# Enigmatisms/NeRF

Hardware: AMD Instinct MI355X
Metric: rays/s (64+128 samples), 800x800 (higher is better)
Workload: dtype bf16

## Files before the change

### include/nerf_amd.h

```cpp
#ifndef NERF_AMD_H
#define NERF_AMD_H

#include <stddef.h>
#include <stdint.h>

#ifdef __cplusplus
extern "C" {
#endif

#define NERF_AMD_OK            0
#define NERF_AMD_EINVAL       -1
#define NERF_AMD_EUNSUPPORTED -2
#define NERF_AMD_EHIP         -3

#define NERF_AMD_F32   0
#define NERF_AMD_BF16  1
#define NERF_AMD_BF16_F8 2

#define NERF_AMD_NET_PROPOSAL 0
#define NERF_AMD_NET_MIP      1
#define NERF_AMD_NET_REF      2
#define NERF_AMD_NET_PROPOSAL_128 3
#define NERF_AMD_PROP_W128 0x100
#define NERF_AMD_NET_MIP_128 4
// ... 100 lines not shown
                      int softplus_density, float blur_alpha, uint64_t rng_seed, int64_t rng_ray_offset,
                      float* z_fine, int64_t* below, float* w_prop, float* z_coarse, void* stream);

int nerf_amd_composite(const float* rgbo, const float* z, int z_stride, const float* dirs, int dirs_stride,
                       int64_t N, int S, int flags, int act, float sigma_shift, float near, float far,
                       const float* normal, const float* cam_dir,
                       float* rgb, float* weights, float* depth, float* normal_img, void* stream);

int nerf_amd_merge_depths(const float* z_fine, const float* z_coarse, int64_t N, int K, int C, float* z_out, void* stream);

int nerf_amd_merge_depths_order(const float* z_fine, const float* z_coarse, const int64_t* f_inds, int64_t N, int K, int C, float* z_out,
                                int64_t* order, int64_t* all_inds, void* stream);

int nerf_amd_coarse_grad_select(const float* grads, const int64_t* sort_inds, int64_t N, int T, int D, int c_pnum, float* out, void* stream);

#define NERF_AMD_DOT_LOSS_WORKSPACE_FLOATS 512
int nerf_amd_weighted_dot_loss(const float* w, const float* a, const float* b, int64_t M, int mode, float scale, float* out, float* workspace, void* stream);
int nerf_amd_weighted_dot_loss_backward(const float* g, const float* w, const float* a, const float* b, int64_t M, int mode, float scale, float* d_w,
                                        float* d_a, float* d_b, void* stream);

#define NERF_AMD_DISTORTION_MAX_S 1024
#define NERF_AMD_DISTORTION_WORKSPACE_FLOATS 4096
int nerf_amd_distortion_loss(const float* w, const float* t, int64_t N, int S, int mode, float scale, float* out, float* workspace, void* stream);
int nerf_amd_distortion_loss_backward(const float* w, const float* t, int64_t N, int S, int mode, float scale, const float* g, float* d_w,
                                      float* d_t, void* stream);

int nerf_amd_mfma_stream(int iters, int workgroups, int mode, float* sink, void* stream);

int nerf_amd_get_bounds(const float* w_prop, const int64_t* below, int64_t N, int C, int K, float* bounds, void* stream);

size_t nerf_amd_train_dump_bytes(int net, int precision, int64_t M);
int nerf_amd_proposal_forward_train(const void* packed, int precision, const nerf_amd_samples* src, float* density, void* dump,
                                    void* stream);
int nerf_amd_mip_forward_train(const void* packed, int precision, const nerf_amd_samples* src, float* rgbo, void* dump, void* stream);
int nerf_amd_train_dump_to_rows(const void* dump, int net, int precision, int64_t M, int layer, int n_features, void* out,
                                void* stream);
int nerf_amd_relu_mask(void* delta, const void* act, int precision, int64_t n, void* stream);
int64_t nerf_amd_relu_mask_bias_partials(int precision, int64_t rows, int cols);
int nerf_amd_relu_mask_bias(void* delta, const void* act, int precision, int64_t rows, int cols, float* col_sum, void* stream);

int64_t nerf_amd_train_dump_rows_mask_partials(void);
int nerf_amd_train_dump_rows_mask(const void* dump, int net, int precision, int64_t M, int layer, int n_features, void* act_out, void* delta,
                                  float* col_sum, void* stream);

int nerf_amd_encode_rows(const float* x, int x_stride, int64_t M, int L, int normalize, int precision, void* out, void* stream);

size_t nerf_amd_packed_backward_bytes(int net, int precision);
int    nerf_amd_pack_weights_backward(int net, int precision, const float* const* weights, int n_tensors, void* packed_bwd, void* stream);
int    nerf_amd_proposal_backward_chain(const void* packed_bwd, int precision, const float* g_density, int64_t M, const void* act_dump,
                                        void* delta_dump, void* stream);
int    nerf_amd_mip_backward_chain(const void* packed_bwd, int precision, const float* g_rgbo, const float* rgbo, int64_t M,
                                   const void* act_dump, void* delta_dump, void* stream);
size_t nerf_amd_weight_grads_workspace_bytes(int net, int precision, int64_t M);
int    nerf_amd_proposal_weight_grads(int precision, int64_t M, const void* act_dump, const void* delta_dump, float* const* d_weights,
                                      float* const* d_biases, void* workspace, void* stream);
int    nerf_amd_mip_weight_grads(int precision, int64_t M, const void* act_dump, const void* delta_dump, const float* const* weights,
                                 const float* const* biases, float* const* d_weights, float* const* d_biases, void* workspace, void* stream);
int    nerf_amd_ref_forward_train_dump(const void* packed, int precision, const nerf_amd_samples* src, int ref_flags, const float* bn_noise,
                                       float* rgbo, float* normal, void* dump, float* aux, void* stream);
int    nerf_amd_ref_forward_train_dump_rng(const void* packed, int precision, const nerf_amd_samples* src, int ref_flags, uint64_t noise_seed,
                                           const uint64_t* noise_seed_dev, float noise_std, float* rgbo, float* normal, void* dump, float* aux,
                                           void* stream);
int    nerf_amd_philox_normal(float* out, int64_t M, uint64_t rng_seed, const uint64_t* seed_dev, float std, int64_t sample_offset, void* stream);
#define NERF_AMD_CONTRACTED 0x100
size_t nerf_amd_density_grad_workspace_bytes(int net, int precision, int64_t M);
int    nerf_amd_density_grad(int net, const void* packed_bwd, int precision, int64_t M, const void* act_dump, const float* x, int x_stride,
                             const float* scale, int scale_stride, float* grad, void* workspace, void* stream);
size_t nerf_amd_ref_backward_workspace_bytes(int precision, int64_t M);
int    nerf_amd_ref_backward(const void* packed_bwd, int precision, int ref_flags, int64_t M, const void* act_dump, const float* aux,
                             const float* dirs, int dir_stride, const float* g_out, int g_stride, const float* ide_table,
                             float* const* d_weights, float* const* d_biases, void* workspace, void* stream);
int    nerf_amd_adam_step(float* const* params, const float* const* grads, float* const* exp_avg, float* const* exp_avg_sq,
                          const int64_t* numel, int n_tensors, float* step, double lr, const double* lr_dev, double beta1, double beta2,
                          double eps, float grad_scale, void* stream);

int nerf_amd_sigma_to_weights_backward(const float* sigma, const float* z, const float* dirs, int64_t N, int S, int act,
                                       const float* d_weights, float* d_sigma, void* stream);
int nerf_amd_composite_backward(const float* rgbo, const float* z, int z_stride, const float* dirs, int dirs_stride, int64_t N, int S,
                                int flags, int act, float sigma_shift, float near, float far, const float* d_rgb,
                                const float* d_weights, const float* d_depth, float* d_rgbo, void* stream);
int nerf_amd_max_blur_backward(const float* weights, const float* d_out, int64_t N, int S, float* d_weights, void* stream);
int nerf_amd_get_bounds_backward(const int64_t* below, const float* d_bounds, int64_t N, int C, int K, float* d_w_prop, void* stream);

size_t nerf_amd_render_workspace_bytes(int64_t N, int n_fine);
int    nerf_amd_render_rays(const void* packed_prop, const void* packed_mip, int precision,
                            const float* rays, const nerf_amd_samples* camera, int64_t ray_offset,
                            const float* z_base, const float* u_strat, const float* u_inv, int64_t N, int n_fine,
                            float near, float far, int white_bkg,
                            float* rgb, float* depth, float* weights, void* workspace, void* stream);

size_t nerf_amd_render_ref_workspace_bytes(int64_t N, int n_fine);
int    nerf_amd_render_rays_ref(const void* packed_prop, const void* packed_ref, int precision, int ref_flags, const float* rays,
                                const nerf_amd_samples* camera, int64_t ray_offset, const float* z_base, const float* u_strat,
                                const float* u_inv, int64_t N, int n_fine, float near, float far, int white_bkg, const float* cam_dir,
                                float* rgb, float* depth, float* normal_img, void* workspace, void* stream);

size_t nerf_amd_gemm_workspace_bytes(int64_t M, int64_t N, int64_t P);
int    nerf_amd_gemm(int precision, int64_t M, int64_t N, int64_t P, const float* A, int64_t a_si, int64_t a_sp,
                     const float* B, int64_t b_sp, int64_t b_sj, float* C, int64_t ldc, const float* bias, int act,
                     const float* mask, int64_t ldm, void* workspace, void* stream);
int    nerf_amd_sigmoid_backward(const float* g, int64_t g_stride, const float* y, int64_t y_stride, int64_t M, int cols,
                                 float* out, int64_t out_stride, void* stream);

int nerf_amd_ref_dir_inputs(const float* heads, int64_t heads_stride, const float* dirs, int64_t dirs_stride, int64_t M, int ide_level,
                            const float* ide_table, float* out, int64_t out_stride, float* normal, void* stream);
int nerf_amd_ref_dir_inputs_backward(const float* heads, int64_t heads_stride, const float* dirs, int64_t dirs_stride, int64_t M, int ide_level,
                                     const float* ide_table, const float* d_out, int64_t d_out_stride, const float* g_normal,
                                     int64_t g_normal_stride, float* d_heads, int64_t d_heads_stride, void* stream);
int nerf_amd_ref_combine(const float* heads, int64_t heads_stride, const float* spec, int64_t spec_stride, int64_t M, int ref_flags,
                         float* rgbo, void* stream);
int nerf_amd_ref_combine_backward(const float* g_rgbo, int64_t g_stride, const float* heads, int64_t heads_stride, const float* spec,
                                  int64_t spec_stride, int64_t M, int ref_flags, float* d_spec, int64_t d_spec_stride, float* d_heads,
                                  int64_t d_heads_stride, void* stream);
int nerf_amd_positional_encoding_backward(const float* d_enc, int64_t d_enc_stride, const float* x, int64_t x_stride, int64_t M, int L,
                                          int cat_origin, float* d_x, void* stream);
int nerf_amd_add_rows(float* dst, int64_t dst_stride, const float* src, int64_t src_stride, int64_t M, int cols, void* stream);
int nerf_amd_contract_positions(const float* x, int64_t x_stride, int64_t M, const float* g, int64_t g_stride, float* out, void* stream);

int nerf_amd_rows_gemm(int64_t M, int64_t N, int64_t K, const void* X, int64_t ldx, const void* W, int64_t ldw, int64_t n_pad,
                       const float* bias, int act, void* C, int64_t ldc, int out_bf16, void* stream);
int nerf_amd_rows_to_bf16(const float* src, int64_t rows_src, int64_t src_stride, int64_t rows, int cols, int fill, void* dst,
                          int64_t dst_stride, void* stream);

#ifdef __cplusplus
}
#endif
#endif
```

### nerf_amd/_lib.py

```python
import ctypes as C
import os

import torch

_HERE = os.path.dirname(os.path.abspath(__file__))
LIB_PATH = os.environ.get("NERF_AMD_LIB") or os.path.join(_HERE, "libnerf_amd.so")

F32, BF16 = 0, 1
BF16_F8 = 2
EXPECTED_VERSION = 125
NET_PROPOSAL, NET_MIP, NET_REF, NET_PROPOSAL_128, NET_MIP_128 = 0, 1, 2, 3, 4
FINE_W128 = 0x200
PROP_W128 = 0x100
ACT_RELU, ACT_IDENTITY, ACT_SOFTPLUS = 0, 1, 2

c_float_p = C.POINTER(C.c_float)
c_void = C.c_void_p
i64 = C.c_int64


class Samples(C.Structure):
    _fields_ = [("mode", C.c_int32), ("S", C.c_int32), ("M", C.c_int64), ("pts", c_void), ("pts_stride", C.c_int32),
                ("z_stride", C.c_int32), ("rays", c_void), ("z", c_void), ("z_base", c_void), ("u", c_void),
                ("z_jitter", C.c_float), ("H", C.c_int32), ("W", C.c_int32), ("fx", C.c_float), ("fy", C.c_float),
# ... 5 lines not shown
    "nerf_amd_last_error": (C.c_char_p, []),
    "nerf_amd_version": (C.c_int, []),
    "nerf_amd_device_info": (C.c_int, [C.POINTER(C.c_int), C.POINTER(C.c_int)]),
    "nerf_amd_packed_bytes": (C.c_size_t, [C.c_int, C.c_int]),
    "nerf_amd_pack_weights": (C.c_int, [C.c_int, C.c_int, C.POINTER(c_void), C.POINTER(c_void), C.c_int, c_void, c_void]),
    "nerf_amd_proposal_forward": (C.c_int, [c_void, C.c_int, C.POINTER(Samples), c_void, c_void]),
    "nerf_amd_mip_forward": (C.c_int, [c_void, C.c_int, C.POINTER(Samples), c_void, c_void]),
    "nerf_amd_mip_forward_composite": (C.c_int, [c_void, C.c_int, C.POINTER(Samples), C.c_int, C.c_float, C.c_float, c_void, c_void, c_void,
                                                 c_void]),
    "nerf_amd_ref_forward": (C.c_int, [c_void, C.c_int, C.POINTER(Samples), C.c_int, c_void, c_void, c_void]),
    "nerf_amd_ref_forward_train": (C.c_int, [c_void, C.c_int, C.POINTER(Samples), C.c_int, c_void, c_void, c_void, c_void]),
    "nerf_amd_positional_encoding": (C.c_int, [c_void, i64, C.c_int, c_void, c_void]),
    "nerf_amd_ipe_feature": (C.c_int, [c_void, c_void, i64, C.c_int, C.c_int, C.c_float, c_void, c_void, c_void, c_void, c_void]),
    "nerf_amd_ipe_feature_contracted": (C.c_int, [c_void, c_void, i64, C.c_int, C.c_int, C.c_float, c_void, c_void, c_void, c_void, c_void]),
    "nerf_amd_cone_parameters": (C.c_int, [c_void, i64, C.c_int, C.c_float, c_void, c_void, c_void, c_void]),
    "nerf_amd_dirs_norm": (C.c_int, [c_void, i64, c_void, c_void]),
    "nerf_amd_generate_rays": (C.c_int, [c_float_p, C.c_int, C.c_int, C.c_float, C.c_float, i64, i64, c_void, c_void]),
    "nerf_amd_length2pts": (C.c_int, [c_void, c_void, i64, C.c_int, c_void, c_void]),
    "nerf_amd_sigma_to_weights": (C.c_int, [c_void, c_void, c_void, i64, C.c_int, C.c_int, c_void, c_void]),
    "nerf_amd_max_blur": (C.c_int, [c_void, i64, C.c_int, C.c_float, c_void, c_void]),
    "nerf_amd_inverse_sample": (C.c_int, [c_void, c_void, c_void, i64, C.c_int, C.c_int, C.c_int, c_void, c_void, c_void]),
    "nerf_amd_sample_pdf": (C.c_int, [c_void, c_void, c_void, i64, C.c_int, C.c_int, c_void, c_void, c_void, c_void]),
    "nerf_amd_pixel_rays": (C.c_int, [c_float_p, C.c_float, C.c_float, c_void, i64, c_void, c_void]),
    "nerf_amd_sample_training_rays": (C.c_int, [c_void, c_void, i64, c_float_p, C.c_float, C.c_float, C.c_float, C.c_float, i64, C.c_int, C.c_uint64,
                                               c_void, c_void, c_void, c_void, c_void]),
    "nerf_amd_sample_training_rays_dev": (C.c_int, [c_void, c_void, i64, c_void, C.c_float, C.c_float, C.c_float, C.c_float, i64, C.c_int, c_void,
                                                   c_void, c_void, c_void, c_void, c_void]),
    "nerf_amd_sample_scene_rays": (C.c_int, [c_void, c_void, i64, C.c_int, C.c_int, c_void, i64, C.c_int, C.c_int, C.c_int, C.c_int, C.c_float, C.c_float,
                                            C.c_float, C.c_float, i64, C.c_int, C.c_uint64, c_void, c_void, c_void, c_void, c_void, c_void, c_void]),
    "nerf_amd_philox_uniforms": (C.c_int, [c_void, i64, C.c_int, C.c_uint64, c_void, c_void]),
    "nerf_amd_philox_stream": (C.c_int, [c_void, i64, C.c_int, C.c_uint64, c_void, i64, C.c_int, c_void]),
    "nerf_amd_advance_seed": (C.c_int, [c_void, c_void]),
    "nerf_amd_stratified_points": (C.c_int, [c_void, c_void, c_void, C.c_float, i64, C.c_int, c_void, c_void, c_void]),
    "nerf_amd_resample": (C.c_int, [c_void, c_void, c_void, c_void, C.c_float, c_void, C.c_int, c_void, i64, C.c_int,
                                    C.c_int, C.c_int, C.c_float, C.c_uint64, i64, c_void, c_void, c_void, c_void, c_void]),
    "nerf_amd_composite": (C.c_int, [c_void, c_void, C.c_int, c_void, C.c_int, i64, C.c_int, C.c_int, C.c_int, C.c_float, C.c_float,
                                     C.c_float, c_void, c_void, c_void, c_void, c_void, c_void, c_void]),
    "nerf_amd_train_dump_rows_mask_partials": (i64, []),
    "nerf_amd_train_dump_rows_mask": (C.c_int, [c_void, C.c_int, C.c_int, i64, C.c_int, C.c_int, c_void, c_void, c_void, c_void]),
    "nerf_amd_render_ref_workspace_bytes": (C.c_size_t, [i64, C.c_int]),
    "nerf_amd_render_rays_ref": (C.c_int, [c_void, c_void, C.c_int, C.c_int, c_void, C.POINTER(Samples), i64, c_void, c_void, c_void, i64, C.c_int,
                                          C.c_float, C.c_float, C.c_int, c_void, c_void, c_void, c_void, c_void, c_void]),
    "nerf_amd_encode_rows": (C.c_int, [c_void, C.c_int, i64, C.c_int, C.c_int, C.c_int, c_void, c_void]),
    "nerf_amd_merge_depths": (C.c_int, [c_void, c_void, i64, C.c_int, C.c_int, c_void, c_void]),
    "nerf_amd_merge_depths_order": (C.c_int, [c_void, c_void, c_void, i64, C.c_int, C.c_int, c_void, c_void, c_void, c_void]),
    "nerf_amd_coarse_grad_select": (C.c_int, [c_void, c_void, i64, C.c_int, C.c_int, C.c_int, c_void, c_void]),
    "nerf_amd_mfma_stream": (C.c_int, [C.c_int, C.c_int, C.c_int, c_void, c_void]),
    "nerf_amd_weighted_dot_loss": (C.c_int, [c_void, c_void, c_void, i64, C.c_int, C.c_float, c_void, c_void, c_void]),
    "nerf_amd_weighted_dot_loss_backward": (C.c_int, [c_void, c_void, c_void, c_void, i64, C.c_int, C.c_float, c_void, c_void, c_void, c_void]),
    "nerf_amd_distortion_loss": (C.c_int, [c_void, c_void, i64, C.c_int, C.c_int, C.c_float, c_void, c_void, c_void]),
    "nerf_amd_distortion_loss_backward": (C.c_int, [c_void, c_void, i64, C.c_int, C.c_int, C.c_float, c_void, c_void, c_void, c_void]),
    "nerf_amd_get_bounds": (C.c_int, [c_void, c_void, i64, C.c_int, C.c_int, c_void, c_void]),
    "nerf_amd_train_dump_bytes": (C.c_size_t, [C.c_int, C.c_int, i64]),
    "nerf_amd_proposal_forward_train": (C.c_int, [c_void, C.c_int, C.POINTER(Samples), c_void, c_void, c_void]),
    "nerf_amd_mip_forward_train": (C.c_int, [c_void, C.c_int, C.POINTER(Samples), c_void, c_void, c_void]),
    "nerf_amd_train_dump_to_rows": (C.c_int, [c_void, C.c_int, C.c_int, i64, C.c_int, C.c_int, c_void, c_void]),
    "nerf_amd_relu_mask": (C.c_int, [c_void, c_void, C.c_int, i64, c_void]),
    "nerf_amd_relu_mask_bias_partials": (i64, [C.c_int, i64, C.c_int]),
    "nerf_amd_relu_mask_bias": (C.c_int, [c_void, c_void, C.c_int, i64, C.c_int, c_void, c_void]),
    "nerf_amd_packed_backward_bytes": (C.c_size_t, [C.c_int, C.c_int]),
    "nerf_amd_pack_weights_backward": (C.c_int, [C.c_int, C.c_int, C.POINTER(c_void), C.c_int, c_void, c_void]),
    "nerf_amd_proposal_backward_chain": (C.c_int, [c_void, C.c_int, c_void, i64, c_void, c_void, c_void]),
    "nerf_amd_mip_backward_chain": (C.c_int, [c_void, C.c_int, c_void, c_void, i64, c_void, c_void, c_void]),
    "nerf_amd_weight_grads_workspace_bytes": (C.c_size_t, [C.c_int, C.c_int, i64]),
    "nerf_amd_proposal_weight_grads": (C.c_int, [C.c_int, i64, c_void, c_void, C.POINTER(c_void), C.POINTER(c_void), c_void, c_void]),
    "nerf_amd_mip_weight_grads": (C.c_int, [C.c_int, i64, c_void, c_void, C.POINTER(c_void), C.POINTER(c_void), C.POINTER(c_void),
                                           C.POINTER(c_void), c_void, c_void]),
    "nerf_amd_ref_forward_train_dump": (C.c_int, [c_void, C.c_int, C.POINTER(Samples), C.c_int, c_void, c_void, c_void, c_void, c_void, c_void]),
    "nerf_amd_ref_forward_train_dump_rng": (C.c_int, [c_void, C.c_int, C.POINTER(Samples), C.c_int, C.c_uint64, c_void, C.c_float, c_void, c_void, c_void,
                                                      c_void, c_void]),
    "nerf_amd_philox_normal": (C.c_int, [c_void, i64, C.c_uint64, c_void, C.c_float, i64, c_void]),
    "nerf_amd_density_grad_workspace_bytes": (C.c_size_t, [C.c_int, C.c_int, i64]),
    "nerf_amd_density_grad": (C.c_int, [C.c_int, c_void, C.c_int, i64, c_void, c_void, C.c_int, c_void, C.c_int, c_void, c_void, c_void]),
    "nerf_amd_ref_backward_workspace_bytes": (C.c_size_t, [C.c_int, i64]),
    "nerf_amd_ref_backward": (C.c_int, [c_void, C.c_int, C.c_int, i64, c_void, c_void, c_void, C.c_int, c_void, C.c_int, c_void, C.POINTER(c_void),
                                       C.POINTER(c_void), c_void, c_void]),
    "nerf_amd_adam_step": (C.c_int, [C.POINTER(c_void), C.POINTER(c_void), C.POINTER(c_void), C.POINTER(c_void), C.POINTER(i64), C.c_int, c_void,
                                    C.c_double, c_void, C.c_double, C.c_double, C.c_double, C.c_float, c_void]),
    "nerf_amd_sigma_to_weights_backward": (C.c_int, [c_void, c_void, c_void, i64, C.c_int, C.c_int, c_void, c_void, c_void]),
    "nerf_amd_composite_backward": (C.c_int, [c_void, c_void, C.c_int, c_void, C.c_int, i64, C.c_int, C.c_int, C.c_int, C.c_float, C.c_float,
                                              C.c_float, c_void, c_void, c_void, c_void, c_void]),
    "nerf_amd_max_blur_backward": (C.c_int, [c_void, c_void, i64, C.c_int, c_void, c_void]),
    "nerf_amd_get_bounds_backward": (C.c_int, [c_void, c_void, i64, C.c_int, C.c_int, c_void, c_void]),
    "nerf_amd_render_workspace_bytes": (C.c_size_t, [i64, C.c_int]),
    "nerf_amd_render_rays": (C.c_int, [c_void, c_void, C.c_int, c_void, C.POINTER(Samples), i64, c_void, c_void, c_void, i64,
                                       C.c_int, C.c_float, C.c_float, C.c_int, c_void, c_void, c_void, c_void, c_void]),
    "nerf_amd_gemm_workspace_bytes": (C.c_size_t, [i64, i64, i64]),
    "nerf_amd_gemm": (C.c_int, [C.c_int, i64, i64, i64, c_void, i64, i64, c_void, i64, i64, c_void, i64, c_void, C.c_int, c_void, i64, c_void, c_void]),
    "nerf_amd_sigmoid_backward": (C.c_int, [c_void, i64, c_void, i64, i64, C.c_int, c_void, i64, c_void]),
    "nerf_amd_ref_dir_inputs": (C.c_int, [c_void, i64, c_void, i64, i64, C.c_int, c_void, c_void, i64, c_void, c_void]),
    "nerf_amd_ref_dir_inputs_backward": (C.c_int, [c_void, i64, c_void, i64, i64, C.c_int, c_void, c_void, i64, c_void, i64, c_void, i64, c_void]),
    "nerf_amd_ref_combine": (C.c_int, [c_void, i64, c_void, i64, i64, C.c_int, c_void, c_void]),
    "nerf_amd_ref_combine_backward": (C.c_int, [c_void, i64, c_void, i64, c_void, i64, i64, C.c_int, c_void, i64, c_void, i64, c_void]),
    "nerf_amd_positional_encoding_backward": (C.c_int, [c_void, i64, c_void, i64, i64, C.c_int, C.c_int, c_void, c_void]),
    "nerf_amd_contract_positions": (C.c_int, [c_void, i64, i64, c_void, i64, c_void, c_void]),
    "nerf_amd_add_rows": (C.c_int, [c_void, i64, c_void, i64, i64, C.c_int, c_void]),
    "nerf_amd_rows_gemm": (C.c_int, [i64, i64, i64, c_void, i64, c_void, i64, i64, c_void, C.c_int, c_void, i64, C.c_int, c_void]),
    "nerf_amd_rows_to_bf16": (C.c_int, [c_void, i64, i64, i64, C.c_int, C.c_int, c_void, i64, c_void]),
}


def _load():
    if not os.path.exists(LIB_PATH):
        raise ImportError(
            "nerf_amd: %s is missing. Build it with `python -c 'import __graft_entry__ as g; g.build()'` "
            "(or `make -C nerf_amd/csrc`). There is no CPU/torch fallback." % LIB_PATH)
    lib = C.CDLL(LIB_PATH)
    for name, (res, args) in SIGNATURES.items():
        fn = getattr(lib, name)
        fn.restype = res
        fn.argtypes = args
    got = lib.nerf_amd_version()
    if got != EXPECTED_VERSION and not os.environ.get("NERF_AMD_LIB"):
        raise ImportError("nerf_amd: %s is ABI version %d, this package expects %d -- rebuild it (`make -C nerf_amd/csrc`)" % (LIB_PATH, got, EXPECTED_VERSION))
    return lib


lib = _load()


class NerfAmdError(RuntimeError):
    pass


def check(rc: int, what: str = ""):
    if rc != 0:
        msg = lib.nerf_amd_last_error()
        raise NerfAmdError("%s failed (%d): %s" % (what or "nerf_amd call", rc, msg.decode() if msg else "?"))
```

### nerf_amd/csrc/capi.hip

```cpp
#include <hip/hip_runtime.h>
#include <stdio.h>
#include <string.h>

#include "../../include/nerf_amd.h"
#include "mlp_layout.h"

int mlp_launch_proposal(const void*, int, const nerf_amd_samples&, float*, hipStream_t);
int mlp_launch_proposal128(const void*, int, const nerf_amd_samples&, float*, hipStream_t);
int mlp_launch_mip(const void*, int, const nerf_amd_samples&, float*, hipStream_t);
int mlp_launch_mip128(const void*, int, const nerf_amd_samples&, float*, hipStream_t);
int mlp_launch_mip_composite(const void*, int, const nerf_amd_samples&, float*, float*, float*, int, float, float, hipStream_t);
int mlp_launch_ref(const void*, int, const nerf_amd_samples&, float*, float*, const float*, int, hipStream_t);
size_t mlp_train_layer_stride(int, int64_t);
size_t mlp_train_mask_stride(int, int64_t);
int mlp_launch_proposal_train(const void*, int, const nerf_amd_samples&, float*, void*, hipStream_t);
int mlp_launch_mip_train(const void*, int, const nerf_amd_samples&, float*, void*, hipStream_t);
int sk_frag_to_rows(const void*, int, int64_t, int, int64_t, void*, hipStream_t);
int sk_relu_mask(void*, const void*, int, int64_t, hipStream_t);
int sk_merge_sorted(const float*, const float*, int64_t, int, int, float*, hipStream_t);
int sk_merge_sorted_order(const float*, const float*, const int64_t*, int64_t, int, int, float*, int64_t*, int64_t*, hipStream_t);
int sk_coarse_grad_select(const float*, const int64_t*, int64_t, int, int, int, float*, hipStream_t);
int pack_mfma_stream(int, int, int, float*, hipStream_t);
int sk_weighted_dot_loss(const float*, const float*, const float*, int64_t, int, float, float*, float*, hipStream_t);
int sk_weighted_dot_loss_backward(const float*, const float*, const float*, const float*, int64_t, int, float, float*, float*, float*, hipStream_t);
int sk_distortion_loss(const float*, const float*, int64_t, int, int, float, float*, float*, hipStream_t);
int sk_distortion_loss_backward(const float*, const float*, int64_t, int, int, float, const float*, float*, float*, hipStream_t);
int sk_encode_rows(const float*, int, int64_t, int, int, int, void*, hipStream_t);
int sk_frag_rows_mask_blocks();
int sk_frag_rows_mask(const void*, int, int64_t, int, int64_t, void*, void*, float*, hipStream_t);
int sk_relu_mask_bias(void*, const void*, int, int64_t, int, float*, hipStream_t);
int pack_ref(int, const float* const*, const float* const*, void*, hipStream_t);
int pack_proposal_bwd(int, const float* const*, void*, hipStream_t);
int pack_mip_bwd(int, const float* const*, void*, hipStream_t);
int pack_ref_bwd(int, const float* const*, void*, hipStream_t);
int mlp_launch_ref_train(const void*, int, const nerf_amd_samples&, float*, float*, const float*, void*, float*, int, hipStream_t, unsigned long long, const unsigned long long*, float);
size_t bwd_density_grad_workspace_bytes(int, int64_t);
int bwd_density_grad(int, const void*, int, int64_t, const void*, const float*, int, const float*, int, float*, void*, hipStream_t, int);
size_t bwd_ref_workspace_bytes(int, int64_t);
int bwd_ref_backward(const void*, int, int64_t, const void*, const float*, const float*, int, const float*, int, const float*, float* const*,
                     float* const*, void*, int, hipStream_t);
int bwd_launch_prop_chain(const void*, int, const float*, int64_t, const void*, void*, hipStream_t);
int bwd_launch_mip_chain(const void*, int, const float*, const float*, int64_t, const void*, void*, hipStream_t);
size_t bwd_wgrad_workspace_bytes(int, int, int64_t);
int bwd_prop_weight_grads(int, int64_t, const void*, const void*, float* const*, float* const*, void*, hipStream_t);
int bwd_mip_weight_grads(int, int64_t, const void*, const void*, const float* const*, const float* const*, float* const*, float* const*, void*,
                         hipStream_t);
int bwd_launch_adam(float* const*, const float* const*, float* const*, float* const*, const long long*, int, float*, double, const double*, double,
                    double, double, float, hipStream_t);
int pack_proposal(int, const float* const*, const float* const*, void*, hipStream_t);
int pack_proposal128(int, const float* const*, const float* const*, void*, hipStream_t);
int pack_mip128(int, const float* const*, const float* const*, void*, hipStream_t);
int pack_mip(int, const float* const*, const float* const*, void*, hipStream_t);
int sk_positional_encoding(const float*, int64_t, int, float*, hipStream_t);
int sk_ipe_feature(const float*, const float*, int64_t, int, int, float, const float*, float*, float*, float*, int, hipStream_t);
int sk_dirs_norm(const float*, int64_t, float*, hipStream_t);
int sk_dirs_norm_scratch(const float*, int64_t, float*, void*, hipStream_t);
int sk_train_sampler(const float*, const int64_t*, int64_t, const float*, const float*, float, float, float, float, int64_t, int, uint64_t, const uint64_t*,
                     float*, float*, float*, float*, hipStream_t);
int sk_scene_sampler(const float*, const float*, int64_t, int, int, const int64_t*, int64_t, int, int, int, int, float, float, float, float, int64_t, int,
                     uint64_t, const uint64_t*, float*, float*, float*, float*, int64_t*, hipStream_t);
int sk_philox_uniforms(float*, int64_t, int, uint64_t, const uint64_t*, int64_t, int, hipStream_t);
int sk_philox_normal(float*, int64_t, uint64_t, const uint64_t*, float, int64_t, hipStream_t);
size_t gk_gemm_workspace_bytes(int64_t, int64_t, int64_t);
int gk_gemm(int, int64_t, int64_t, int64_t, const float*, int64_t, int64_t, const float*, int64_t, int64_t, float*, int64_t, const float*, int, const float*, int64_t,
            void*, hipStream_t);
int gk_sigmoid_backward(const float*, int64_t, const float*, int64_t, int64_t, int, float*, int64_t, hipStream_t);
int gr_dir_inputs(const float*, int64_t, const float*, int64_t, int64_t, int, const float*, float*, int64_t, float*, hipStream_t);
int gr_dir_inputs_backward(const float*, int64_t, const float*, int64_t, int64_t, int, const float*, const float*, int64_t, const float*, int64_t, float*, int64_t,
                           hipStream_t);
int gr_combine(const float*, int64_t, const float*, int64_t, int64_t, int, float*, hipStream_t);
int gr_combine_backward(const float*, int64_t, const float*, int64_t, const float*, int64_t, int64_t, int, float*, int64_t, float*, int64_t, hipStream_t);
int gr_pe_backward(const float*, int64_t, const float*, int64_t, int64_t, int, int, float*, hipStream_t);
int gr_add_rows(float*, int64_t, const float*, int64_t, int64_t, int, hipStream_t);
int gr_contract(const float*, int64_t, int64_t, const float*, int64_t, float*, hipStream_t);
int rg_rows_gemm(int64_t, int64_t, int64_t, const void*, int64_t, const void*, int64_t, int64_t, const float*, int, void*, int64_t, int, hipStream_t);
int rg_rows_to_bf16(const float*, int64_t, int64_t, int64_t, int, int, void*, int64_t, hipStream_t);
int sk_advance_seed(uint64_t*, hipStream_t);
int sk_cone_parameters(const float*, int64_t, int, float, float*, float*, float*, hipStream_t);
int sk_generate_rays(const float*, int, int, float, float, int64_t, int64_t, float*, hipStream_t);
int sk_length2pts(const float*, const float*, int64_t, int, float*, hipStream_t);
int sk_sigma_to_weights(const float*, const float*, const float*, int64_t, int, int, float*, hipStream_t);
int sk_max_blur(const float*, int64_t, int, float, float*, hipStream_t);
int sk_inverse_sample(const float*, const float*, const float*, int64_t, int, int, int, int, float*, int64_t*, int64_t*, hipStream_t);
int sk_pixel_rays(const float*, float, float, const int64_t*, int64_t, float*, hipStream_t);
int sk_stratified_points(const float*, const float*, const float*, float, int64_t, int, float*, float*, hipStream_t);
int sk_resample(const float*, const float*, const float*, const float*, float, const float*, int, const float*, int64_t, int,
                int, int, float, uint64_t, int64_t, float*, int64_t*, float*, float*, hipStream_t);
int sk_composite(const float*, const float*, int, const float*, int, int64_t, int, int, int, float, float, float, const float*,
                 const float*, float*, float*, float*, float*, hipStream_t);
int sk_get_bounds(const float*, const int64_t*, int64_t, int, int, float*, hipStream_t);
int sk_weights_backward(const float*, int, int, const float*, int, const float*, int, int64_t, int, int, int, float, const float*, const float*,
                        const float*, const float*, int, float, float, float*, int, int, float*, hipStream_t);
int sk_max_blur_backward(const float*, const float*, int64_t, int, float*, hipStream_t);
int sk_get_bounds_backward(const int64_t*, const float*, int64_t, int, int, float*, hipStream_t);

namespace {
thread_local char g_err[512] = "";

int fail(int code, const char* fmt, const char* a = "") {
    snprintf(g_err, sizeof(g_err), fmt, a);
    return code;
}
int hip_status(int e, const char* where) {
    if (e == 0) return NERF_AMD_OK;
    snprintf(g_err, sizeof(g_err), "%s: HIP error %d (%s)", where, e, hipGetErrorString((hipError_t)e));
    return NERF_AMD_EHIP;
}
inline hipStream_t S(void* s) { return reinterpret_cast<hipStream_t>(s); }

int check_samples(const nerf_amd_samples* s, bool need_dir) {
    if (!s) return fail(NERF_AMD_EINVAL, "samples descriptor is NULL");
    if (s->M < 0) return fail(NERF_AMD_EINVAL, "negative sample count");
    if (s->mode == 0) {
        if (!s->pts && s->M) return fail(NERF_AMD_EINVAL, "mode 0 needs pts");
        if (s->pts_stride < (need_dir ? 6 : 3)) return fail(NERF_AMD_EINVAL, "pts_stride too small for this network");
    } else if (s->mode == 1 || s->mode == 2) {
        if (s->S <= 0) return fail(NERF_AMD_EINVAL, "S must be positive");
        if (s->mode == 1 && !s->rays && s->M) return fail(NERF_AMD_EINVAL, "mode 1 needs rays");
        if (s->mode == 2 && (s->H <= 0 || s->W <= 0)) return fail(NERF_AMD_EINVAL, "mode 2 needs H, W");
        if (!s->z && !s->z_base && s->M) return fail(NERF_AMD_EINVAL, "need z, or z_base (with u, or without: in-kernel uniforms from rng_seed)");
    } else {
        return fail(NERF_AMD_EINVAL, "unknown sample mode");
    }
    if (s->ipe) {
        if (!need_dir) return fail(NERF_AMD_EUNSUPPORTED, "integrated PE is wired for the MipNeRF kernel only");
        if (s->mode != 1 || !s->z || s->z_stride < s->S + 1) return fail(NERF_AMD_EINVAL, "integrated PE needs mode 1 with S+1 depths per ray (z, z_stride > S)");
        if (!s->ipe_dir_norm || !(s->ipe_radius > 0.0f)) return fail(NERF_AMD_EINVAL, "integrated PE needs ipe_dir_norm (device) and a positive ipe_radius");
    }
    return NERF_AMD_OK;
}
bool bad_prec(int p) { return p != NERF_AMD_F32 && p != NERF_AMD_BF16; }
int check_distortion(int64_t N, int Sn, int mode) {
    if (N < 0) return fail(NERF_AMD_EINVAL, "negative ray count");
    if (mode != 0 && mode != 1) return fail(NERF_AMD_EINVAL, "unknown mode (0: Regularizer, 1: Mip-NeRF 360 L_dist)");
    if (Sn < 2 || Sn > NERF_AMD_DISTORTION_MAX_S) return fail(NERF_AMD_EINVAL, "bad size (S must be 2..1024 depths per row: a ray's rows live in LDS)");
    return NERF_AMD_OK;
}
}

extern "C" {

const char* nerf_amd_last_error(void) { return g_err; }
int nerf_amd_version(void) { return 125; }

int nerf_amd_device_info(int* n_cu, int* arch_is_gfx950) {
    int dev = 0;
    hipDeviceProp_t p;
    int e = (int)hipGetDevice(&dev);
    if (!e) e = (int)hipGetDeviceProperties(&p, dev);
    if (e) return hip_status(e, "nerf_amd_device_info");
    if (n_cu) *n_cu = p.multiProcessorCount;
    if (arch_is_gfx950) *arch_is_gfx950 = strncmp(p.gcnArchName, "gfx950", 6) == 0;
    return NERF_AMD_OK;
}

size_t nerf_amd_packed_bytes(int net, int precision) {
    if (bad_prec(precision)) return 0;
    if (net == NERF_AMD_NET_PROPOSAL) return PropLayout::packed_bytes(precision);
    if (net == NERF_AMD_NET_MIP) return MipLayout::packed_bytes(precision);
    if (net == NERF_AMD_NET_REF) return RefLayout::packed_bytes(precision);
    if (net == NERF_AMD_NET_PROPOSAL_128) return PropLayout128::packed_bytes(precision);
    if (net == NERF_AMD_NET_MIP_128) return MipLayout128::packed_bytes(precision);
    return 0;
}
static int launch_mip_any(int flags, const void* packed, int precision, const nerf_amd_samples& s, float* rgbo, hipStream_t st) {
    return (flags & NERF_AMD_FINE_W128) ? mlp_launch_mip128(packed, precision, s, rgbo, st) : mlp_launch_mip(packed, precision, s, rgbo, st);
}
static int launch_proposal_any(int flags, const void* packed, int precision, const nerf_amd_samples& s, float* density, hipStream_t st) {
    return (flags & NERF_AMD_PROP_W128) ? mlp_launch_proposal128(packed, precision, s, density, st) : mlp_launch_proposal(packed, precision, s, density, st);
}

int nerf_amd_pack_weights(int net, int precision, const float* const* weights, const float* const* biases, int n_tensors,
                          void* packed, void* stream) {
    if (bad_prec(precision)) return fail(NERF_AMD_EINVAL, "unknown precision");
    if (!weights || !biases || !packed) return fail(NERF_AMD_EINVAL, "NULL argument");
    const int want = (net == NERF_AMD_NET_PROPOSAL || net == NERF_AMD_NET_PROPOSAL_128) ? 5
                     : ((net == NERF_AMD_NET_MIP || net == NERF_AMD_NET_MIP_128) ? 11 : (net == NERF_AMD_NET_REF ? 20 : -1));
// ... 146 lines not shown
    if (!pose_host || (N && (!rgbs || !coords || !rgb || !rays))) return fail(NERF_AMD_EINVAL, "NULL argument");
    if ((pts == nullptr) != (lengths == nullptr) || (pts && C < 1)) return fail(NERF_AMD_EINVAL, "pts and lengths go together (C >= 1)");
    return hip_status(sk_train_sampler(rgbs, coords, n_pixels, pose_host, nullptr, fx, fy, near, far, N, C, rng_seed, nullptr, pts, lengths, rgb, rays, S(stream)),
                      "nerf_amd_sample_training_rays");
}
int nerf_amd_sample_training_rays_dev(const float* rgbs, const int64_t* coords, int64_t n_pixels, const float* pose_dev, float fx, float fy,
                                      float near, float far, int64_t N, int C, const uint64_t* seed_dev, float* pts, float* lengths, float* rgb,
                                      float* rays, void* stream) {
    if (N < 0 || C < 0 || n_pixels < 1) return fail(NERF_AMD_EINVAL, "bad size");
    if (!pose_dev || !seed_dev || (N && (!rgbs || !coords || !rgb || !rays))) return fail(NERF_AMD_EINVAL, "NULL argument");
    if ((pts == nullptr) != (lengths == nullptr) || (pts && C < 1)) return fail(NERF_AMD_EINVAL, "pts and lengths go together (C >= 1)");
    return hip_status(sk_train_sampler(rgbs, coords, n_pixels, nullptr, pose_dev, fx, fy, near, far, N, C, 0, seed_dev, pts, lengths, rgb, rays, S(stream)),
                      "nerf_amd_sample_training_rays_dev");
}
int nerf_amd_sample_scene_rays(const float* images, const float* poses, int64_t V, int H, int W, const int64_t* view_ids, int64_t K, int x0, int x1,
                               int y0, int y1, float fx, float fy, float near, float far, int64_t N, int C, uint64_t rng_seed,
                               const uint64_t* seed_dev, float* pts, float* lengths, float* rgb, float* rays, int64_t* index, void* stream) {
    if (!images) return fail(NERF_AMD_EINVAL, "nerf_amd_sample_scene_rays: images is NULL");
    if (!poses) return fail(NERF_AMD_EINVAL, "nerf_amd_sample_scene_rays: poses is NULL");
    if (V < 1 || H < 1 || W < 1) return fail(NERF_AMD_EINVAL, "nerf_amd_sample_scene_rays: V, H, W must be positive");
    if (K < 1 || (!view_ids && K > V)) return fail(NERF_AMD_EINVAL, "nerf_amd_sample_scene_rays: need 1 <= K (and K <= V without view_ids)");
    if (x0 < 0 || x1 > W || x0 >= x1) return fail(NERF_AMD_EINVAL, "nerf_amd_sample_scene_rays: window x0, x1 empty or outside the image (0 <= x0 < x1 <= W)");
    if (y0 < 0 || y1 > H || y0 >= y1) return fail(NERF_AMD_EINVAL, "nerf_amd_sample_scene_rays: window y0, y1 empty or outside the image (0 <= y0 < y1 <= H)");
    if (N < 0) return fail(NERF_AMD_EINVAL, "nerf_amd_sample_scene_rays: N is negative");
    if (C < 0) return fail(NERF_AMD_EINVAL, "nerf_amd_sample_scene_rays: C is negative");
    if (pts && !lengths) return fail(NERF_AMD_EINVAL, "nerf_amd_sample_scene_rays: pts given without lengths");
    if (lengths && C > 0 && !pts) return fail(NERF_AMD_EINVAL, "nerf_amd_sample_scene_rays: lengths given without pts");
    if (!rgb) return fail(NERF_AMD_EINVAL, "nerf_amd_sample_scene_rays: rgb is NULL");
    if (!rays) return fail(NERF_AMD_EINVAL, "nerf_amd_sample_scene_rays: rays is NULL");
    if (N == 0) return NERF_AMD_OK;
    return hip_status(sk_scene_sampler(images, poses, V, H, W, view_ids, K, x0, x1, y0, y1, fx, fy, near, far, N, C, rng_seed, seed_dev, pts, lengths, rgb,
                                       rays, index, S(stream)),
                      "nerf_amd_sample_scene_rays");
}
int nerf_amd_philox_uniforms(float* out, int64_t N, int K, uint64_t rng_seed, const uint64_t* seed_dev, void* stream) {
    if (N < 0 || K < 0) return fail(NERF_AMD_EINVAL, "negative size");
    if (N * K && !out) return fail(NERF_AMD_EINVAL, "NULL argument");
    return hip_status(sk_philox_uniforms(out, N, K, rng_seed, seed_dev, 0, 0, S(stream)), "nerf_amd_philox_uniforms");
}
int nerf_amd_philox_stream(float* out, int64_t N, int K, uint64_t rng_seed, const uint64_t* seed_dev, int64_t ray_offset, int stream_id, void* stream) {
    if (N < 0 || K < 0 || ray_offset < 0) return fail(NERF_AMD_EINVAL, "negative size");
    if (stream_id != NERF_AMD_PHILOX_INV && stream_id != NERF_AMD_PHILOX_STRAT) return fail(NERF_AMD_EINVAL, "unknown stream_id");
    if (stream_id == NERF_AMD_PHILOX_STRAT && K > 64) return fail(NERF_AMD_EINVAL, "the stratified stream has 64 slots per ray");
    if (N * K && !out) return fail(NERF_AMD_EINVAL, "NULL argument");
    return hip_status(sk_philox_uniforms(out, N, K, rng_seed, seed_dev, ray_offset, stream_id == NERF_AMD_PHILOX_STRAT, S(stream)), "nerf_amd_philox_stream");
}
int nerf_amd_advance_seed(uint64_t* seed_dev, void* stream) {
    if (!seed_dev) return fail(NERF_AMD_EINVAL, "NULL argument");
    return hip_status(sk_advance_seed(seed_dev, S(stream)), "nerf_amd_advance_seed");
}

int nerf_amd_stratified_points(const float* rays, const float* z_base, const float* u, float z_jitter, int64_t N, int Sn,
                               float* z_out, float* pts, void* stream) {
    if (N < 0 || Sn < 0) return fail(NERF_AMD_EINVAL, "negative size");
    if (N * Sn && (!z_base || !u || !z_out || (pts && !rays))) return fail(NERF_AMD_EINVAL, "NULL argument");
    return hip_status(sk_stratified_points(rays, z_base, u, z_jitter, N, Sn, z_out, pts, S(stream)), "nerf_amd_stratified_points");
}

int nerf_amd_resample(const float* density, const float* z, const float* z_base, const float* u_strat, float z_jitter,
                      const float* dirs, int dirs_stride, const float* u_inv, int64_t N, int C, int K, int softplus_density,
                      float blur_alpha, uint64_t rng_seed, int64_t rng_ray_offset, float* z_fine, int64_t* below, float* w_prop,
                      float* z_coarse, void* stream) {
    if (N < 0 || C < 3 || C > 256 || K < 1 || K > 1024) return fail(NERF_AMD_EINVAL, "need 3 <= C <= 256 and 1 <= K <= 1024");
    if (N && (!density || !dirs || !z_fine)) return fail(NERF_AMD_EINVAL, "NULL argument");
    if (N && !z && !z_base) return fail(NERF_AMD_EINVAL, "need z, or z_base (with u_strat, or without: in-kernel uniforms)");
    return hip_status(sk_resample(density, z, z_base, u_strat, z_jitter, dirs, dirs_stride, u_inv, N, C, K, softplus_density,
                                  blur_alpha, rng_seed, rng_ray_offset, z_fine, below, w_prop, z_coarse, S(stream)), "nerf_amd_resample");
}

int nerf_amd_composite(const float* rgbo, const float* z, int z_stride, const float* dirs, int dirs_stride, int64_t N, int Sn,
                       int flags, int act, float sigma_shift, float near, float far, const float* normal, const float* cam_dir, float* rgb,
                       float* weights, float* depth, float* normal_img, void* stream) {
    if (N < 0 || Sn < 1 || act < 0 || act > 2 || z_stride < Sn) return fail(NERF_AMD_EINVAL, "bad size, stride or activation");
    if (N && (!rgbo || !z || !dirs || !rgb)) return fail(NERF_AMD_EINVAL, "NULL argument");
    if (normal_img && !(normal && cam_dir)) return fail(NERF_AMD_EINVAL, "normal_img needs normal and cam_dir");
    return hip_status(sk_composite(rgbo, z, z_stride, dirs, dirs_stride, N, Sn, flags, act, sigma_shift, near, far, normal, cam_dir,
                                   rgb, weights, depth, normal_img, S(stream)), "nerf_amd_composite");
}

int nerf_amd_get_bounds(const float* w_prop, const int64_t* below, int64_t N, int C, int K, float* bounds, void* stream) {
    if (N < 0 || C < 1 || C > 4096 || K < 2) return fail(NERF_AMD_EINVAL, "bad size");
    if (N && (!w_prop || !below || !bounds)) return fail(NERF_AMD_EINVAL, "NULL argument");
    return hip_status(sk_get_bounds(w_prop, below, N, C, K, bounds, S(stream)), "nerf_amd_get_bounds");
}

int nerf_amd_merge_depths(const float* z_fine, const float* z_coarse, int64_t N, int K, int C, float* z_out, void* stream) {
    if (N < 0 || K < 1 || C < 1 || K + C > 2048) return fail(NERF_AMD_EINVAL, "bad size (K + C <= 2048: four rays of depths and their sort scratch per workgroup live in 64 KiB of LDS)");
    if (N && (!z_fine || !z_coarse || !z_out)) return fail(NERF_AMD_EINVAL, "NULL argument");
    return hip_status(sk_merge_sorted(z_fine, z_coarse, N, K, C, z_out, S(stream)), "nerf_amd_merge_depths");
}

int nerf_amd_merge_depths_order(const float* z_fine, const float* z_coarse, const int64_t* f_inds, int64_t N, int K, int C, float* z_out, int64_t* order,
                                int64_t* all_inds, void* stream) {
    if (N < 0 || K < 1 || C < 1 || K + C > 1024) return fail(NERF_AMD_EINVAL, "bad size (K + C <= 1024: four rays of depths, indices and their sort scratch per workgroup live in 64 KiB of LDS)");
    if (N && (!z_fine || !z_coarse || !z_out || !order)) return fail(NERF_AMD_EINVAL, "NULL argument");
    if (N && all_inds && !f_inds) return fail(NERF_AMD_EINVAL, "all_inds needs f_inds");
    return hip_status(sk_merge_sorted_order(z_fine, z_coarse, f_inds, N, K, C, z_out, order, all_inds, S(stream)), "nerf_amd_merge_depths_order");
}

int nerf_amd_coarse_grad_select(const float* grads, const int64_t* sort_inds, int64_t N, int T, int D, int c_pnum, float* out, void* stream) {
    if (N < 0 || T < 1 || D < 1 || c_pnum < 0 || c_pnum > T) return fail(NERF_AMD_EINVAL, "bad size");
    if (N && c_pnum && (!grads || !sort_inds || !out)) return fail(NERF_AMD_EINVAL, "NULL argument");
    return hip_status(sk_coarse_grad_select(grads, sort_inds, N, T, D, c_pnum, out, S(stream)), "nerf_amd_coarse_grad_select");
}

int nerf_amd_weighted_dot_loss(const float* w, const float* a, const float* b, int64_t M, int mode, float scale, float* out, float* workspace, void* stream) {
    if (M < 0 || (mode != 0 && mode != 1)) return fail(NERF_AMD_EINVAL, "bad size / mode");
    if (!out || !workspace || (M && (!w || !a || !b))) return fail(NERF_AMD_EINVAL, "NULL argument");
    return hip_status(sk_weighted_dot_loss(w, a, b, M, mode, scale, out, workspace, S(stream)), "nerf_amd_weighted_dot_loss");
}

int nerf_amd_weighted_dot_loss_backward(const float* g, const float* w, const float* a, const float* b, int64_t M, int mode, float scale, float* d_w,
                                        float* d_a, float* d_b, void* stream) {
    if (M < 0 || (mode != 0 && mode != 1)) return fail(NERF_AMD_EINVAL, "bad size / mode");
    if (M && (!g || !w || !a || !b)) return fail(NERF_AMD_EINVAL, "NULL argument");
    return hip_status(sk_weighted_dot_loss_backward(g, w, a, b, M, mode, scale, d_w, d_a, d_b, S(stream)), "nerf_amd_weighted_dot_loss_backward");
}

int nerf_amd_distortion_loss(const float* w, const float* t, int64_t N, int Sn, int mode, float scale, float* out, float* workspace, void* stream) {
    if (int e = check_distortion(N, Sn, mode)) return e;
    if (!out || !workspace || (N && (!w || !t))) return fail(NERF_AMD_EINVAL, "NULL argument");
    return hip_status(sk_distortion_loss(w, t, N, Sn, mode, scale, out, workspace, S(stream)), "nerf_amd_distortion_loss");
}

int nerf_amd_distortion_loss_backward(const float* w, const float* t, int64_t N, int Sn, int mode, float scale, const float* g, float* d_w, float* d_t,
                                      void* stream) {
    if (int e = check_distortion(N, Sn, mode)) return e;
    if (N && (!w || !t || !g)) return fail(NERF_AMD_EINVAL, "NULL argument");
    return hip_status(sk_distortion_loss_backward(w, t, N, Sn, mode, scale, g, d_w, d_t, S(stream)), "nerf_amd_distortion_loss_backward");
}

int nerf_amd_mfma_stream(int iters, int workgroups, int mode, float* sink, void* stream) {
    if (iters < 0 || workgroups < 1 || mode < 0 || mode > 3 || !sink) return fail(NERF_AMD_EINVAL, "bad argument");
    return hip_status(pack_mfma_stream(iters, workgroups, mode, sink, S(stream)), "nerf_amd_mfma_stream");
}

static int train_layers(int net) {
    return net == NERF_AMD_NET_PROPOSAL ? PROP_DUMP_SLOTS : (net == NERF_AMD_NET_MIP ? MIP_DUMP_SLOTS : (net == NERF_AMD_NET_REF ? REF_DUMP_SLOTS : 0));
}
static bool bad_train_prec(int p, int net = NERF_AMD_NET_MIP) {
    return p != NERF_AMD_F32 && p != NERF_AMD_BF16 && !(p == NERF_AMD_BF16_F8 && net != NERF_AMD_NET_REF);
}
size_t nerf_amd_train_dump_bytes(int net, int precision, int64_t M) {
    if (M < 0 || !train_layers(net) || bad_train_prec(precision, net)) return 0;
    const size_t bits = (size_t)train_layers(net) * mlp_train_mask_stride(precision, M);
    return (size_t)train_layers(net) * mlp_train_layer_stride(precision, M) + bits;
}
int nerf_amd_proposal_forward_train(const void* packed, int precision, const nerf_amd_samples* src, float* density, void* dump, void* stream) {
    if (!packed || !src || !dump) return fail(NERF_AMD_EINVAL, "NULL argument");
    if (bad_train_prec(precision)) return fail(NERF_AMD_EINVAL, "bad precision");
    if (src->M && !density) return fail(NERF_AMD_EINVAL, "NULL output");
    if (int c = check_samples(src, false)) return c;
    return hip_status(mlp_launch_proposal_train(packed, precision, *src, density, dump, S(stream)), "nerf_amd_proposal_forward_train");
}
int nerf_amd_mip_forward_train(const void* packed, int precision, const nerf_amd_samples* src, float* rgbo, void* dump, void* stream) {
    if (!packed || !src || !dump) return fail(NERF_AMD_EINVAL, "NULL argument");
    if (bad_train_prec(precision)) return fail(NERF_AMD_EINVAL, "bad precision");
    if (src->M && !rgbo) return fail(NERF_AMD_EINVAL, "NULL output");
    if (int c = check_samples(src, true)) return c;
    return hip_status(mlp_launch_mip_train(packed, precision, *src, rgbo, dump, S(stream)), "nerf_amd_mip_forward_train");
}
int nerf_amd_train_dump_to_rows(const void* dump, int net, int precision, int64_t M, int layer, int n_features, void* out, void* stream) {
    if (M < 0 || layer < 0 || layer >= train_layers(net) || n_features < 16 || n_features > 256 || (n_features & 15))
        return fail(NERF_AMD_EINVAL, "bad layer or feature count");
    if (M && (!dump || !out)) return fail(NERF_AMD_EINVAL, "NULL argument");
    const size_t stride = mlp_train_layer_stride(precision, M);
// ... 443 lines not shown
```

### nerf_amd/csrc/sample_kernels.hip

```cpp
#include "device_common.h"
#include "host_common.h"
#include "../../include/nerf_amd.h"

extern __shared__ __attribute__((aligned(16))) char smem[];

namespace {

constexpr int WAVES_PER_BLOCK = 4;

DEVINL int wave_in_block() { return (int)(threadIdx.x >> 6); }

constexpr int ENC_TILE = 64;
static inline size_t enc_lds_bytes(int L) { return (size_t)ENC_TILE * (6 * L + 6) * 4; }
template <bool IPE, class Moments>
DEVINL void encode_tile(float (*mom)[6], float* stage, int64_t base, int64_t total, int L, float* __restrict__ feat, Moments&& moments) {
    const int width = 6 * L, pairs_per = 3 * L;
    const int nsamp = (int)(total - base < ENC_TILE ? total - base : ENC_TILE);
    if ((int)threadIdx.x < nsamp) moments((int)threadIdx.x, base + threadIdx.x);
    __syncthreads();
    const int n_pairs = nsamp * pairs_per;
    for (int p = threadIdx.x; p < n_pairs; p += blockDim.x) {
        const int sl = p / pairs_per, rem = p - sl * pairs_per;
        const int l = rem / 3, c = rem - 3 * l;
        float sn, cs;
        sincos_quadrant(mom[sl][c] * (float)(1 << l), sn, cs);
        if (IPE) {
            const float e = expf(-0.5f * (mom[sl][3 + c] * (float)(1u << (2 * l))));
            sn *= e; cs *= e;
        }
        stage[sl * width + 6 * l + c] = sn;
        stage[sl * width + 6 * l + 3 + c] = cs;
    }
    __syncthreads();
    const int cnt = nsamp * width;
    float* o = feat + base * width;
    const f32x4* s4 = reinterpret_cast<const f32x4*>(stage);
    f32x4* o4 = reinterpret_cast<f32x4*>(o);
    for (int i = threadIdx.x; i < cnt / 4; i += blockDim.x) o4[i] = s4[i];
    for (int i = (cnt & ~3) + threadIdx.x; i < cnt; i += blockDim.x) o[i] = stage[i];
    __syncthreads();
}

__global__ __launch_bounds__(256) void pe_kernel(const float* __restrict__ x, int64_t M, int L, float* __restrict__ out) {
    float* stage = reinterpret_cast<float*>(smem);
    float (*mom)[6] = reinterpret_cast<float (*)[6]>(stage + ENC_TILE * 6 * L);
    for (int64_t base = blockIdx.x * (int64_t)ENC_TILE; base < M; base += (int64_t)gridDim.x * ENC_TILE)
        encode_tile<false>(mom, stage, base, M, L, out, [&](int sl, int64_t m) {
            mom[sl][0] = x[m * 3]; mom[sl][1] = x[m * 3 + 1]; mom[sl][2] = x[m * 3 + 2];
        });
}

__global__ __launch_bounds__(256) void ipe_feature_kernel(const float* __restrict__ z, const float* __restrict__ rays, int64_t N, int S, int L,
                                                           float r2, const float* __restrict__ dir_norm, float* __restrict__ feat,
                                                           float* __restrict__ mu_out, float* __restrict__ mu_t_out, int contract) {
    float* stage = reinterpret_cast<float*>(smem);
    float (*mom)[6] = reinterpret_cast<float (*)[6]>(stage + ENC_TILE * 6 * L);
    const int64_t total = N * S;
    const float dn = dir_norm[0];
    for (int64_t base = blockIdx.x * (int64_t)ENC_TILE; base < total; base += (int64_t)gridDim.x * ENC_TILE)
        encode_tile<true>(mom, stage, base, total, L, feat, [&](int sl, int64_t m) {
            const int64_t n = m / S;
            const int si = (int)(m - n * S);
            const float* zz = z + n * (S + 1) + si;
            const ConeMoments c = cone_moments(zz[0], zz[1], r2);
            const float* ry = rays + n * 6;
#pragma unroll
            for (int k = 0; k < 3; ++k) cone_mean_cov(c, ry[k], ry[3 + k], dn, mom[sl][k], mom[sl][3 + k]);
            if (contract) {
                const float nn = norm3(mom[sl][0], mom[sl][1], mom[sl][2]);
                if (nn > 1.0f) {
                    const float kk = (2.0f - 1.0f / nn) / nn;
                    mom[sl][0] *= kk; mom[sl][1] *= kk; mom[sl][2] *= kk;
                }
            }
            if (mu_out) { mu_out[m * 3] = mom[sl][0]; mu_out[m * 3 + 1] = mom[sl][1]; mu_out[m * 3 + 2] = mom[sl][2]; }
            if (mu_t_out) mu_t_out[m] = c.mu_t;
        });
}

__global__ void cone_parameters_kernel(const float* __restrict__ z, int64_t N, int S, float r2, float* __restrict__ mu_t, float* __restrict__ var_t,
                                       float* __restrict__ var_r) {
    const int64_t total = N * S;
    for (int64_t m = blockIdx.x * (int64_t)blockDim.x + threadIdx.x; m < total; m += (int64_t)gridDim.x * blockDim.x) {
        const int64_t n = m / S;
        const float* zz = z + n * (S + 1) + (m - n * S);
        const ConeMoments c = cone_moments(zz[0], zz[1], r2);
        mu_t[m] = c.mu_t; var_t[m] = c.var_t; var_r[m] = c.var_r;
    }
}

__global__ __launch_bounds__(1024) void dirs_norm_kernel(const float* __restrict__ rays, int64_t N, float* __restrict__ out) {
    __shared__ double part[1024];
    double acc = 0.0;
// ... 106 lines not shown
        const Philox4 r = philox4x32_10((uint32_t)n, (uint32_t)((uint64_t)n >> 32), (uint32_t)(sidx >> 2), PHILOX_STREAM_TRAIN, (uint32_t)seed,
                                        (uint32_t)(seed >> 32));
        const int w = sidx & 3;
        const float u = u01_from_bits(w == 0 ? r.w[0] : (w == 1 ? r.w[1] : (w == 2 ? r.w[2] : r.w[3])));
        const float z = (near + (float)sidx * res) + u * res;
        lengths[n * C + sidx] = z;
        const float* q = ray_s[rl];
        float* o = pts + (n * C + sidx) * 3;
        o[0] = q[0] + q[3] * z; o[1] = q[1] + q[4] * z; o[2] = q[2] + q[5] * z;
    }
}
__global__ __launch_bounds__(256) void train_sampler_kernel(const float* __restrict__ rgbs, const int64_t* __restrict__ coords, int64_t P, Cam cam,
                                                            float near, float res, int64_t N, int C, uint64_t seed, float* __restrict__ pts,
                                                            float* __restrict__ lengths, float* __restrict__ rgb, float* __restrict__ rays,
                                                            const float* __restrict__ pose_dev, const uint64_t* __restrict__ seed_dev) {
    __shared__ float ray_s[4][6];
    if (pose_dev != nullptr) {
#pragma unroll
        for (int i = 0; i < 12; ++i) cam.pose[i] = pose_dev[i];
    }
    if (seed_dev != nullptr) seed = seed_dev[0];
    for (int64_t n0 = blockIdx.x * (int64_t)4; n0 < N; n0 += (int64_t)gridDim.x * 4) {
        __syncthreads();
        if (threadIdx.x < 4 && n0 + threadIdx.x < N) {
            const int64_t n = n0 + threadIdx.x;
            const int64_t idx = (int64_t)__umul64hi(sampler_index_word(n, seed), (uint64_t)P);
            sampler_ray(cam.pose, cam.fx, cam.fy, (float)coords[idx * 2], (float)coords[idx * 2 + 1], ray_s[threadIdx.x], rays + n * 6);
#pragma unroll
            for (int k = 0; k < 3; ++k) rgb[n * 3 + k] = rgbs[idx * 3 + k];
        }
        __syncthreads();
        if (lengths == nullptr) continue;
        sampler_samples(n0, N, C, seed, near, res, ray_s, lengths, pts);
    }
}

__global__ __launch_bounds__(256) void scene_sampler_kernel(const float* __restrict__ images, const float* __restrict__ poses, int64_t V, int H, int W,
                                                            const int64_t* __restrict__ view_ids, int64_t K, int x0, int ww, int y0, int64_t wp,
                                                            float fx, float fy, float near, float res, int64_t N, int C, uint64_t seed,
                                                            const uint64_t* __restrict__ seed_dev, float* __restrict__ pts, float* __restrict__ lengths,
                                                            float* __restrict__ rgb, float* __restrict__ rays, int64_t* __restrict__ index) {
    __shared__ float ray_s[4][6];
    if (seed_dev != nullptr) seed = seed_dev[0];
    const uint64_t P = (uint64_t)K * (uint64_t)wp;
    for (int64_t n0 = blockIdx.x * (int64_t)4; n0 < N; n0 += (int64_t)gridDim.x * 4) {
        __syncthreads();
        if (threadIdx.x < 4 && n0 + threadIdx.x < N) {
            const int64_t n = n0 + threadIdx.x;
            const int64_t cell = (int64_t)__umul64hi(sampler_index_word(n, seed), P);
            const int64_t k = cell / wp, r = cell - k * wp;
            const int64_t wr = r / ww;
            const int64_t row = y0 + wr, col = x0 + (r - wr * ww);
            const int64_t v = view_ids != nullptr ? view_ids[k] : k;
            float* q = ray_s[threadIdx.x];
            if (v >= 0 && v < V) {
                sampler_ray(poses + v * 12, fx, fy, (float)(col - W / 2), (float)(H / 2 - row), q, rays + n * 6);
                const float* px = images + ((v * 3) * (int64_t)H + row) * W + col;
#pragma unroll
                for (int c = 0; c < 3; ++c) rgb[n * 3 + c] = px[(int64_t)c * H * W];
                if (index != nullptr) index[n] = (v * H + row) * W + col;
            } else {
                const float nan = __builtin_nanf("");
#pragma unroll
                for (int c = 0; c < 6; ++c) { q[c] = nan; rays[n * 6 + c] = nan; }
#pragma unroll
                for (int c = 0; c < 3; ++c) rgb[n * 3 + c] = nan;
                if (index != nullptr) index[n] = -1;
            }
        }
        __syncthreads();
        if (lengths == nullptr) continue;
        sampler_samples(n0, N, C, seed, near, res, ray_s, lengths, pts);
    }
}

__global__ void length2pts_kernel(const float* __restrict__ rays, const float* __restrict__ z, int64_t N, int S,
                                  float* __restrict__ out) {
    const int64_t total = N * S * 6;
    for (int64_t i = blockIdx.x * (int64_t)blockDim.x + threadIdx.x; i < total; i += (int64_t)gridDim.x * blockDim.x) {
        const int64_t ns = i / 6;
        const int k = (int)(i - ns * 6);
        const int64_t n = ns / S;
        const float* r = rays + n * 6;
        out[i] = (k < 3) ? (r[k] + r[3 + k] * z[ns]) : r[k];
    }
}

__global__ __launch_bounds__(256) void sigma_to_weights_kernel(const float* __restrict__ sigma, const float* __restrict__ z,
                                                              const float* __restrict__ dirs, int64_t N, int S, int act,
                                                              float* __restrict__ w) {
    for (int64_t n = blockIdx.x * (int64_t)WAVES_PER_BLOCK + wave_in_block(); n < N; n += (int64_t)gridDim.x * WAVES_PER_BLOCK) {
        float nrm = 1.0f;
        const bool scale = dirs != nullptr;
        if (scale) nrm = norm3(dirs[n * 3], dirs[n * 3 + 1], dirs[n * 3 + 2]);
        const float* sg = sigma + n * S;
        const float* zz = z + n * S;
        float* wo = w + n * S;
        wave_sigma_to_weights(S, act, [&](int s) { return sg[s]; },
                              [&](int s) { return scale ? zz[s] * nrm : zz[s]; },
                              [&](int s, float wv, float) { wo[s] = wv; });
    }
}

__global__ void max_blur_kernel(const float* __restrict__ w, int64_t N, int S, float alpha, float* __restrict__ out) {
    const int64_t total = N * S;
    for (int64_t i = blockIdx.x * (int64_t)blockDim.x + threadIdx.x; i < total; i += (int64_t)gridDim.x * blockDim.x) {
        const int s = (int)(i % S);
        const float c = w[i];
        const float front = (s == 0) ? c : fmaxf(w[i - 1], c);
        const float rear = (s == S - 1) ? c : fmaxf(c, w[i + 1]);
        out[i] = 0.5f * (front + rear) + alpha;
    }
}

DEVINL void lds_wave_sync() {
    __builtin_amdgcn_fence(__ATOMIC_RELEASE, "workgroup");
    __builtin_amdgcn_wave_barrier();
    __builtin_amdgcn_fence(__ATOMIC_ACQUIRE, "workgroup");
}

#ifndef SORT_NB_DEF
#define SORT_NB_DEF 256
#define SORT_CAP_DEF 6
#endif
constexpr int SORT_NB = SORT_NB_DEF, SORT_CAP = SORT_CAP_DEF, SORT_PER_LANE = SORT_NB / 64;
constexpr int SORT_LDS_FLOATS = 2 * SORT_NB + SORT_NB * SORT_CAP / 2;

template <class UF>
DEVINL void wave_inverse_sample(const float* pw, const float* bins, int nw, float* cdf, float* samp, int* bel, int* sortbuf,
                                UF&& uf, int K, int sort, float* __restrict__ z_out,
                                int64_t* __restrict__ below_out, int64_t* __restrict__ above_out) {
    const int lane = lane_id();
    const int nb = nw + 1;
    float* part8 = reinterpret_cast<float*>(sortbuf);
    const int nv = nw >> 3;
    if (lane < 8) {
        const int n4 = nv >> 2;
        float a0 = 0.0f, a1 = 0.0f, a2 = 0.0f, a3 = 0.0f;
        for (int i = 0; i < n4; ++i) {
            a0 += pw[32 * i + lane] + 1e-5f;
            a1 += pw[32 * i + 8 + lane] + 1e-5f;
            a2 += pw[32 * i + 16 + lane] + 1e-5f;
            a3 += pw[32 * i + 24 + lane] + 1e-5f;
        }
        for (int v = 4 * n4; v < nv; ++v) a0 += pw[8 * v + lane] + 1e-5f;
        a0 += a1; a0 += a2; a0 += a3;
        part8[lane] = a0;
    }
    lds_wave_sync();
    float total = 0.0f;
    if (nv > 0) {
        for (int j = 8 * nv; j < nw; ++j) total += pw[j] + 1e-5f;
#pragma unroll
        for (int c = 0; c < 8; ++c) total += part8[c];
    } else {
        float a1 = 0.0f, a2 = 0.0f, a3 = 0.0f;
        if (nw >= 4) { total += pw[0] + 1e-5f; a1 += pw[1] + 1e-5f; a2 += pw[2] + 1e-5f; a3 += pw[3] + 1e-5f; }
        for (int j = nw & ~3; j < nw; ++j) total += pw[j] + 1e-5f;
        total += a1; total += a2; total += a3;
    }
    double carry = 0.0;
    if (lane == 0) cdf[0] = 0.0f;
    for (int base = 0; base < nw; base += 64) {
        const int j = base + lane;
        double p = 0.0;
        if (j < nw) p = (double)((pw[j] + 1e-5f) / total);
        const double incl = wave_incl_scan_add(p);
        if (j < nw) cdf[1 + j] = (float)(carry + incl);
        carry += wave_last(incl);
    }
    lds_wave_sync();
    const int halvings = 32 - __builtin_clz((unsigned)nb);
    for (int k0 = 0, i0 = 0; k0 < K; k0 += 192, i0 += 3) {
        float uu[3]; int lo[3], hi[3];
#pragma unroll
        for (int q = 0; q < 3; ++q) {
            const int k = k0 + 64 * q + lane;
            uu[q] = (k < K) ? uf(i0 + q, k) : 0.0f;
            lo[q] = 0; hi[q] = (k < K) ? nb : 0;
        }
        for (int it = 0; it < halvings; ++it) {
#pragma unroll
            for (int q = 0; q < 3; ++q) {
                const int mid = (lo[q] + hi[q]) >> 1;
                const bool open_ = lo[q] < hi[q];
                const float c = cdf[open_ ? mid : 0];
                if (open_) { if (c <= uu[q]) lo[q] = mid + 1; else hi[q] = mid; }
            }
        }
#pragma unroll
        for (int q = 0; q < 3; ++q) {
            const int k = k0 + 64 * q + lane;
            if (k >= K) continue;
            const int below = lo[q] - 1 > 0 ? lo[q] - 1 : 0;
            const int above = lo[q] < nb - 1 ? lo[q] : nb - 1;
            const float c0 = cdf[below], c1 = cdf[above];
            float denom = c1 - c0;
            if (denom < 1e-5f) denom = 1.0f;
            const float t = (uu[q] - c0) / denom;
            const float b0 = bins[below], b1 = bins[above];
            const float v = b0 + t * (b1 - b0);
            if (sort) { samp[k] = v; bel[k] = below; }
            else {
                z_out[k] = v;
                if (below_out) below_out[k] = below;
                if (above_out) above_out[k] = above;
            }
        }
    }
    if (!sort) return;
    lds_wave_sync();
    int* cnt = sortbuf;
    int* pre = sortbuf + SORT_NB;
    unsigned short* mem = reinterpret_cast<unsigned short*>(sortbuf + 2 * SORT_NB);
    for (int b = lane; b < SORT_NB; b += 64) cnt[b] = 0;
    lds_wave_sync();
    int overflow = 0;
    for (int j = lane; j + 1 < nb; j += 64) overflow |= (bins[j + 1] < bins[j]) ? 1 : 0;
    for (int k = lane, i = 0; k < K; k += 64, ++i) {
        int b = (int)(uf(i, k) * (float)SORT_NB);
        b = b < 0 ? 0 : (b > SORT_NB - 1 ? SORT_NB - 1 : b);
        const int pos = atomicAdd(&cnt[b], 1);
        if (pos < SORT_CAP) mem[b * SORT_CAP + pos] = (unsigned short)k; else overflow = 1;
    }
    lds_wave_sync();
    if (__any(overflow)) {
        for (int k = lane; k < K; k += 64) {
            const float v = samp[k];
            int rank = 0;
            for (int j = 0; j < K; ++j) {
                const float o = samp[j];
                rank += (o < v || (o == v && j < k)) ? 1 : 0;
            }
            z_out[rank] = v;
            if (below_out) below_out[rank] = bel[k];
        }
        return;
    }
    {
        int c[SORT_PER_LANE], tot = 0;
#pragma unroll
        for (int i = 0; i < SORT_PER_LANE; ++i) { c[i] = cnt[lane * SORT_PER_LANE + i]; tot += c[i]; }
        int run = wave_incl_scan_add(tot) - tot;
#pragma unroll
        for (int i = 0; i < SORT_PER_LANE; ++i) { pre[lane * SORT_PER_LANE + i] = run; run += c[i]; }
    }
    lds_wave_sync();
    for (int k0 = 0, i0 = 0; k0 < K; k0 += 192, i0 += 3) {
        float v[3]; int rank[3], cntb[3], bb[3];
#pragma unroll
        for (int q = 0; q < 3; ++q) {
            const int k = k0 + 64 * q + lane;
            const bool ok = k < K;
            int b = ok ? (int)(uf(i0 + q, k) * (float)SORT_NB) : 0;
            b = b < 0 ? 0 : (b > SORT_NB - 1 ? SORT_NB - 1 : b);
            bb[q] = b;
            v[q] = samp[ok ? k : 0];
            rank[q] = pre[b];
            cntb[q] = ok ? cnt[b] : 0;
        }
        int most = cntb[0] > cntb[1] ? cntb[0] : cntb[1];
        most = most > cntb[2] ? most : cntb[2];
        const int trips = wave_max_i(most);
        for (int p = 0; p < trips; ++p) {
#pragma unroll
            for (int q = 0; q < 3; ++q) {
                const int k = k0 + 64 * q + lane;
                const bool live = p < cntb[q];
                const int jx = mem[bb[q] * SORT_CAP + p];
                const float o = samp[live ? jx : 0];
                rank[q] += (live && (o < v[q] || (o == v[q] && jx < k))) ? 1 : 0;
            }
        }
#pragma unroll
        for (int q = 0; q < 3; ++q) {
            const int k = k0 + 64 * q + lane;
            if (k >= K) continue;
            z_out[rank[q]] = v[q];
            if (below_out) below_out[rank[q]] = bel[k];
        }
    }
}

DEVINL size_t inv_lds_floats(int C, int K) { return (size_t)3 * C + 2 * K + SORT_LDS_FLOATS; }

__global__ __launch_bounds__(256) void inverse_sample_kernel(const float* __restrict__ w, const float* __restrict__ z,
                                                            const float* __restrict__ u, int64_t N, int C, int K, int sort,
                                                            int mode, float* __restrict__ z_out, int64_t* __restrict__ below,
                                                            int64_t* __restrict__ above) {
    float* base = reinterpret_cast<float*>(smem) + wave_in_block() * inv_lds_floats(C, K);
    float* pw = base; float* bins = pw + C; float* cdf = bins + C; float* samp = cdf + C;
    int* bel = reinterpret_cast<int*>(samp + K);
    int* sortbuf = bel + K;
    const int lane = lane_id();
    const int nw = mode == 0 ? C - 2 : C - 1;
    const int wstride = mode == 0 ? C : C - 1;
    for (int64_t n = blockIdx.x * (int64_t)WAVES_PER_BLOCK + wave_in_block(); n < N; n += (int64_t)gridDim.x * WAVES_PER_BLOCK) {
        lds_wave_sync();
        if (mode == 0) {
            for (int j = lane; j < nw; j += 64) pw[j] = w[n * wstride + 1 + j];
            for (int j = lane; j < nw + 1; j += 64) bins[j] = 0.5f * (z[n * C + j + 1] + z[n * C + j]);
        } else {
            for (int j = lane; j < nw; j += 64) pw[j] = w[n * wstride + j];
            for (int j = lane; j < nw + 1; j += 64) bins[j] = z[n * C + j];
        }
        lds_wave_sync();
        const float* un = u + n * K;
        wave_inverse_sample(pw, bins, nw, cdf, samp, bel, sortbuf, [&](int, int k) { return un[k]; }, K, sort, z_out + n * K,
                            below ? below + n * K : nullptr, above ? above + n * K : nullptr);
    }
}

struct ResampleArgs {
    const float* density; const float* z; const float* z_base; const float* u_strat; float z_jitter;
    const float* dirs; int dirs_stride; const float* u_inv; int64_t N; int C; int K; int softplus; float alpha;
    float* z_fine; int64_t* below; float* w_prop; float* z_coarse;
    uint64_t rng_seed; int64_t rng_ray_offset;
};

#ifndef RS_BLOCKS_PER_CU
#define RS_BLOCKS_PER_CU 5
#endif
__global__ __launch_bounds__(256) __attribute__((amdgpu_waves_per_eu(RS_BLOCKS_PER_CU, RS_BLOCKS_PER_CU))) void resample_kernel(ResampleArgs a) {
    const int C = a.C, K = a.K;
    float* base = reinterpret_cast<float*>(smem) + wave_in_block() * (inv_lds_floats(C, K) + 2 * C);
    float* pw = base; float* bins = pw + C; float* cdf = bins + C; float* samp = cdf + C;
    int* bel = reinterpret_cast<int*>(samp + K);
    int* sortbuf = bel + K;
    float* zl = reinterpret_cast<float*>(sortbuf + SORT_LDS_FLOATS);
    float* wraw = zl + C;
    const int lane = lane_id();
    struct RayIn { float dx, dy, dz, zv0, zv1, dens0, dens1, u0, u1, u2; };
    const bool fits = C <= 128 && K <= 192;
    auto load_in = [&](int64_t n) -> RayIn {
        RayIn r;
        const float* dd = a.dirs + n * a.dirs_stride;
        r.dx = dd[0]; r.dy = dd[1]; r.dz = dd[2];
        Philox4 blk = {{0u, 0u, 0u, 0u}};
        const bool draw = !a.u_inv || (!a.z && !a.u_strat);
        if (draw) blk = philox_ray_block(a.rng_seed, n + a.rng_ray_offset, lane);
        auto depth_of = [&](int j, bool first) {
            if (a.z) return a.z[n * C + j];
            const float uu = a.u_strat ? a.u_strat[n * C + j] : (first ? u01_from_bits(blk.w[0]) : philox_u_strat(a.rng_seed, n + a.rng_ray_offset, j));
            return a.z_base[j] + uu * a.z_jitter;
        };
        r.zv0 = r.zv1 = r.dens0 = r.dens1 = 0.0f;
        if (lane < C) { r.zv0 = depth_of(lane, true); r.dens0 = a.density[n * C + lane]; }
        if (lane + 64 < C) { r.zv1 = depth_of(lane + 64, false); r.dens1 = a.density[n * C + lane + 64]; }
        if (a.u_inv) {
            const float* un = a.u_inv + n * K;
            r.u0 = (lane < K) ? un[lane] : 0.0f;
            r.u1 = (lane + 64 < K) ? un[lane + 64] : 0.0f;
            r.u2 = (lane + 128 < K) ? un[lane + 128] : 0.0f;
        } else {
            r.u0 = u01_from_bits(blk.w[1]); r.u1 = u01_from_bits(blk.w[2]); r.u2 = u01_from_bits(blk.w[3]);
        }
        return r;
    };
    const int64_t stride = (int64_t)gridDim.x * WAVES_PER_BLOCK;
    int64_t n = blockIdx.x * (int64_t)WAVES_PER_BLOCK + wave_in_block();
    if (n >= a.N) return;
    RayIn cur = {};
    if (fits) cur = load_in(n);
    for (; n < a.N; n += stride) {
        RayIn nxt = cur;
        if (fits && n + stride < a.N) nxt = load_in(n + stride);
        lds_wave_sync();
// ... 89 lines not shown
        double p = 1.0;
        if (s < S) {
            const float delta = (s + 1 < S) ? (nx - zn[k]) : 1e10f;
            const float m = expf(-density_act(r.c[k][3] + a.sigma_shift, a.act) * delta);
            w = 1.0f - m; p = (double)(m + 1e-10f);
        }
        const double incl = wave_incl_scan_mul(p);
        const double excl = wave_shift_up1(incl, 1.0);
        w *= (float)(carry * excl);
        carry *= wave_last(incl);
        if (s < S) {
            accr += w * r.c[k][0]; accg += w * r.c[k][1]; accb += w * r.c[k][2]; accw += w; accd += w * zn[k];
            if (wout) wout[s] = w;
        }
    }
    accr = wave_sum(accr); accg = wave_sum(accg); accb = wave_sum(accb); accw = wave_sum(accw); accd = wave_sum(accd);
    if (lane == 0) {
        if (a.flags & 2) { const float bg = 1.0f - accw; accr += bg; accg += bg; accb += bg; }
        a.rgb[n * 3] = accr; a.rgb[n * 3 + 1] = accg; a.rgb[n * 3 + 2] = accb;
        if (a.depth) a.depth[n] = (accd - a.near) / (a.far - a.near);
    }
}
template <int NCH>
DEVINL void composite_rays_fast(const CompositeArgs& a, int lane) {
    const int64_t stride = (int64_t)gridDim.x * WAVES_PER_BLOCK;
    int64_t n = blockIdx.x * (int64_t)WAVES_PER_BLOCK + wave_in_block();
    if (n >= a.N) return;
    RayRecs<NCH> cur = load_ray<NCH>(a, n, lane);
    for (; n < a.N; n += stride) {
        RayRecs<NCH> nxt = cur;
        if (n + stride < a.N) nxt = load_ray<NCH>(a, n + stride, lane);
        composite_ray_fast<NCH>(a, n, cur, lane);
        cur = nxt;
    }
}

__global__ __launch_bounds__(256) void composite_kernel(CompositeArgs a) {
    const int S = a.S;
    const int lane = lane_id();
    if (S <= 256 && a.normal == nullptr && a.normal_img == nullptr) {
        if (S <= 128) composite_rays_fast<2>(a, lane);
        else composite_rays_fast<4>(a, lane);
        return;
    }
    for (int64_t n = blockIdx.x * (int64_t)WAVES_PER_BLOCK + wave_in_block(); n < a.N; n += (int64_t)gridDim.x * WAVES_PER_BLOCK) {
        const float* dd = a.dirs + n * a.dirs_stride;
        const bool mul = (a.flags & 1) != 0;
        const float nrm = mul ? norm3(dd[0], dd[1], dd[2]) : 1.0f;
        const float* zz = a.z + n * a.z_stride;
        const f32x4* px = reinterpret_cast<const f32x4*>(a.rgbo) + n * S;
        float accr = 0.0f, accg = 0.0f, accb = 0.0f, accw = 0.0f, accd = 0.0f, accn = 0.0f;
        float cx = 0.0f, cy = 0.0f, cz = 0.0f;
        if (a.normal_img) { cx = a.cam_dir[0]; cy = a.cam_dir[1]; cz = a.cam_dir[2]; }
        float* wout = a.weights ? a.weights + n * S : nullptr;
        const float* nm = a.normal ? a.normal + n * S * 3 : nullptr;
        const float shift = a.sigma_shift;
        wave_sigma_to_weights(S, a.act, [&](int s) { return px[s][3] + shift; },
                              [&](int s) { return mul ? zz[s] * nrm : zz[s]; },
                              [&](int s, float w, float zn) {
                                  const f32x4 c = px[s];
                                  accr += w * c[0]; accg += w * c[1]; accb += w * c[2];
                                  accw += w; accd += w * zn;
                                  if (nm) accn += w * ((nm[s * 3] * cx + nm[s * 3 + 1] * cy) + nm[s * 3 + 2] * cz);
                                  if (wout) wout[s] = w;
                              });
        accr = wave_sum(accr); accg = wave_sum(accg); accb = wave_sum(accb); accw = wave_sum(accw);
        accd = wave_sum(accd);
        if (a.normal_img) accn = wave_sum(accn);
        if (lane == 0) {
            if (a.flags & 2) { const float bg = 1.0f - accw; accr += bg; accg += bg; accb += bg; }
            a.rgb[n * 3] = accr; a.rgb[n * 3 + 1] = accg; a.rgb[n * 3 + 2] = accb;
            if (a.depth) a.depth[n] = (accd - a.near) / (a.far - a.near);
            if (a.normal_img) a.normal_img[n] = (accn + 1.0f) * 0.5f;
        }
    }
}

__global__ __launch_bounds__(256) void get_bounds_kernel(const float* __restrict__ w, const int64_t* __restrict__ below,
                                                        int64_t N, int C, int K, float* __restrict__ bounds) {
    float* sat = reinterpret_cast<float*>(smem) + wave_in_block() * (C + 1);
    const int lane = lane_id();
    for (int64_t n = blockIdx.x * (int64_t)WAVES_PER_BLOCK + wave_in_block(); n < N; n += (int64_t)gridDim.x * WAVES_PER_BLOCK) {
        lds_wave_sync();
        double carry = 0.0;
        if (lane == 0) sat[0] = 0.0f;
        for (int base = 0; base < C; base += 64) {
            const int j = base + lane;
            const double p = (j < C) ? (double)w[n * C + j] : 0.0;
            const double incl = wave_incl_scan_add(p);
            if (j < C) sat[1 + j] = (float)(carry + incl);
            carry += wave_last(incl);
        }
        lds_wave_sync();
        const int64_t* bl = below + n * K;
        for (int k = lane; k < K - 1; k += 64) {
            const int st = (int)bl[k], en = (int)bl[k + 1] + 1;
            bounds[n * (K - 1) + k] = sat[en] - sat[st];
        }
    }
}

constexpr int BWD_MAX_CHUNKS = 16;
struct WeightsBwdArgs {
    const float* sigma; int sigma_stride;
    int sigma_off;
    const float* z; int z_stride; const float* dirs; int dirs_stride; int64_t N; int S; int mul_norm; int act; float sigma_shift;
    const float* rgbo; const float* d_rgb; const float* d_weights; const float* d_depth; int white_bkg; float near, far;
    float* d_sigma; int d_sigma_stride; int d_sigma_off; float* d_rgbo;
};
DEVINL float density_act_grad(float x, int act) {
    if (act == 0) return x > 0.0f ? 1.0f : 0.0f;
    if (act == 2) return x > 20.0f ? 1.0f : 1.0f / (1.0f + expf(-x));
    return 1.0f;
}
template <int BWD_CHUNKS>
__global__ __launch_bounds__(256) void weights_backward_kernel(WeightsBwdArgs a) {
    const int S = a.S;
    const int lane = lane_id();
    for (int64_t n = blockIdx.x * (int64_t)WAVES_PER_BLOCK + wave_in_block(); n < a.N; n += (int64_t)gridDim.x * WAVES_PER_BLOCK) {
        float nrm = 1.0f;
        if (a.mul_norm && a.dirs) { const float* dd = a.dirs + n * a.dirs_stride; nrm = norm3(dd[0], dd[1], dd[2]); }
        const float* zz = a.z + n * a.z_stride;
        float dr = 0.0f, dg = 0.0f, db = 0.0f, dd_ = 0.0f;
        if (a.d_rgb) { dr = a.d_rgb[n * 3]; dg = a.d_rgb[n * 3 + 1]; db = a.d_rgb[n * 3 + 2]; }
        if (a.d_depth) dd_ = a.d_depth[n] / (a.far - a.near);
        const float bg = (a.white_bkg && a.d_rgb) ? ((dr + dg) + db) : 0.0f;
        float m[BWD_CHUNKS], T[BWD_CHUNKS], G[BWD_CHUNKS], delta[BWD_CHUNKS], x[BWD_CHUNKS];
        double carry = 1.0, gw_carry = 0.0;
        double P[BWD_CHUNKS];
#pragma unroll
        for (int c = 0; c < BWD_CHUNKS; ++c) {
            const int s = c * 64 + lane;
            const bool ok = s < S;
            m[c] = 1.0f; T[c] = 0.0f; G[c] = 0.0f; delta[c] = 0.0f; x[c] = 0.0f;
            double p = 1.0;
            float zn0 = 0.0f;
            if (c * 64 < S) {
                if (ok) {
                    zn0 = zz[s] * nrm;
                    delta[c] = (s + 1 < S) ? (zz[s + 1] * nrm - zn0) : 1e10f;
                    x[c] = a.sigma[(n * S + s) * a.sigma_stride + a.sigma_off] + a.sigma_shift;
                    m[c] = expf(-density_act(x[c], a.act) * delta[c]);
                    p = (double)(m[c] + 1e-10f);
                }
                const double incl = wave_incl_scan_mul(p);
                const double excl = wave_shift_up1(incl, 1.0);
                T[c] = (float)(carry * excl);
                carry *= wave_last(incl);
                float g = 0.0f;
                if (ok) {
                    if (a.d_weights) g += a.d_weights[n * S + s];
                    if (a.rgbo) {
                        const float* cc = a.rgbo + (n * S + s) * 4;
                        g += ((dr * cc[0] + dg * cc[1]) + db * cc[2]) - bg;
                    }
                    g += dd_ * zn0;
                }
                G[c] = g;
                const float w = (1.0f - m[c]) * T[c];
                const double gi = wave_incl_scan_add(ok ? (double)(g * w) : 0.0);
                P[c] = gw_carry + gi;
                gw_carry += wave_last(gi);
                if (ok && a.d_rgbo) {
                    float* o = a.d_rgbo + (n * S + s) * 4;
                    o[0] = w * dr; o[1] = w * dg; o[2] = w * db;
                }
            }
        }
        const double total = gw_carry;
#pragma unroll
        for (int c = 0; c < BWD_CHUNKS; ++c) {
            const int s = c * 64 + lane;
            if (s < S) {
                const float suffix = (float)(total - P[c]);
                const float dm = -G[c] * T[c] + suffix / (m[c] + 1e-10f);
                const float ds = dm * (-delta[c] * m[c]) * density_act_grad(x[c], a.act);
                a.d_sigma[(n * S + s) * a.d_sigma_stride + a.d_sigma_off] = ds;
            }
        }
    }
}

__global__ void max_blur_backward_kernel(const float* __restrict__ w, const float* __restrict__ g, int64_t N, int S, float* __restrict__ dw) {
    const int64_t total = N * S;
    for (int64_t i = blockIdx.x * (int64_t)blockDim.x + threadIdx.x; i < total; i += (int64_t)gridDim.x * blockDim.x) {
        const int s = (int)(i % S);
        const float c = w[i];
        float acc = 0.0f;
        if (s == 0) acc += 0.5f * g[i];
        if (s == S - 1) acc += 0.5f * g[i];
        if (s + 1 < S) {
            const float o = w[i + 1];
            const float share = c > o ? 1.0f : (c == o ? 0.5f : 0.0f);
            acc += share * (0.5f * g[i] + 0.5f * g[i + 1]);
        }
        if (s >= 1) {
            const float o = w[i - 1];
            const float share = c > o ? 1.0f : (c == o ? 0.5f : 0.0f);
            acc += share * (0.5f * g[i - 1] + 0.5f * g[i]);
        }
        dw[i] = acc;
    }
}

__global__ __launch_bounds__(256) void get_bounds_backward_kernel(const int64_t* __restrict__ below, const float* __restrict__ g, int64_t N, int C,
                                                                  int K, float* __restrict__ dw) {
    int* bl_lds = reinterpret_cast<int*>(smem) + wave_in_block() * (2 * K);
    float* g_lds = reinterpret_cast<float*>(bl_lds + K);
    const int lane = lane_id();
    for (int64_t n = blockIdx.x * (int64_t)WAVES_PER_BLOCK + wave_in_block(); n < N; n += (int64_t)gridDim.x * WAVES_PER_BLOCK) {
        lds_wave_sync();
        for (int k = lane; k < K; k += 64) {
            int b = (int)below[n * K + k];
            bl_lds[k] = b < 0 ? 0 : (b > C ? C : b);
            g_lds[k] = (k < K - 1) ? g[n * (K - 1) + k] : 0.0f;
        }
        lds_wave_sync();
        for (int j = lane; j < C; j += 64) {
            float acc = 0.0f;
            for (int k = 0; k < K - 1; ++k) {
                const int st = bl_lds[k];
                int en = bl_lds[k + 1] + 1;
                en = en > C ? C : en;
                if (j >= st && j < en) acc += g_lds[k];
                else if (j >= en && j < st) acc -= g_lds[k];
            }
            dw[n * C + j] = acc;
        }
    }
}

template <int ELEM>
__global__ __launch_bounds__(256) void frag_to_rows_kernel(const char* __restrict__ frag, int64_t n_sub, int n_kg, int64_t M,
                                                           char* __restrict__ out, int ld) {
    const int lane = lane_id(), h = lane >> 5, j = lane & 31;
    constexpr int BLOCK = 512 * ELEM;
    const int row_bytes = n_kg * 16 * ELEM;
    const int pitch = row_bytes + 16;
    char* tile = smem + (size_t)wave_in_block() * 32 * pitch;
    for (int64_t sub = blockIdx.x * (int64_t)WAVES_PER_BLOCK + wave_in_block(); sub < n_sub; sub += (int64_t)gridDim.x * WAVES_PER_BLOCK) {
        lds_wave_sync();
        char* trow = tile + j * pitch;
        for (int kg = 0; kg < n_kg; ++kg) {
            const char* blk = frag + ((size_t)sub * 16 + kg) * BLOCK;
            if constexpr (ELEM == 2) {
                const f32x4 v = *reinterpret_cast<const f32x4*>(blk + lane * 16);
                f32x2 lo = {v[0], v[1]}, hi = {v[2], v[3]};
                *reinterpret_cast<f32x2*>(trow + (16 * kg + 4 * h) * 2) = lo;
                *reinterpret_cast<f32x2*>(trow + (16 * kg + 8 + 4 * h) * 2) = hi;
            } else {
                *reinterpret_cast<f32x4*>(trow + (16 * kg + 4 * h) * 4) = *reinterpret_cast<const f32x4*>(blk + lane * 16);
                *reinterpret_cast<f32x4*>(trow + (16 * kg + 8 + 4 * h) * 4) = *reinterpret_cast<const f32x4*>(blk + 1024 + lane * 16);
            }
        }
        lds_wave_sync();
        const int chunks_per_row = row_bytes / 16;
        const int total = 32 * chunks_per_row;
        char* obase = out + (size_t)sub * 32 * ld * ELEM;
        for (int c = lane; c < total; c += 64) {
            const int r = c / chunks_per_row, q = c - r * chunks_per_row;
            if (sub * 32 + r < M)
                *reinterpret_cast<f32x4*>(obase + (size_t)r * ld * ELEM + q * 16) = *reinterpret_cast<const f32x4*>(tile + r * pitch + q * 16);
        }
    }
}

template <int ELEM>
__global__ __launch_bounds__(256) void frag_rows_mask_kernel(const char* __restrict__ frag, int64_t n_sub, int n_kg, int64_t M,
                                                             char* __restrict__ act_out, char* __restrict__ delta, float* __restrict__ col_sum) {
    const int lane = lane_id(), h = lane >> 5, j = lane & 31;
    constexpr int BLOCK = 512 * ELEM;
    constexpr int NV = 16 / ELEM;
    const int row_bytes = n_kg * 16 * ELEM;
    const int pitch = row_bytes + 16;
    const int ld = n_kg * 16;
    char* tile = smem + (size_t)wave_in_block() * 32 * pitch;
    const int cpr = row_bytes / 16;
    const int q = lane % cpr, r0 = lane / cpr, rstep = 64 / cpr;
    float acc[NV];
#pragma unroll
    for (int e = 0; e < NV; ++e) acc[e] = 0.0f;
    for (int64_t sub = blockIdx.x * (int64_t)WAVES_PER_BLOCK + wave_in_block(); sub < n_sub; sub += (int64_t)gridDim.x * WAVES_PER_BLOCK) {
        lds_wave_sync();
        char* trow = tile + j * pitch;
        for (int kg = 0; kg < n_kg; ++kg) {
            const char* blk = frag + ((size_t)sub * 16 + kg) * BLOCK;
            if constexpr (ELEM == 2) {
                const f32x4 v = *reinterpret_cast<const f32x4*>(blk + lane * 16);
                f32x2 lo = {v[0], v[1]}, hi = {v[2], v[3]};
                *reinterpret_cast<f32x2*>(trow + (16 * kg + 4 * h) * 2) = lo;
                *reinterpret_cast<f32x2*>(trow + (16 * kg + 8 + 4 * h) * 2) = hi;
            } else {
                *reinterpret_cast<f32x4*>(trow + (16 * kg + 4 * h) * 4) = *reinterpret_cast<const f32x4*>(blk + lane * 16);
                *reinterpret_cast<f32x4*>(trow + (16 * kg + 8 + 4 * h) * 4) = *reinterpret_cast<const f32x4*>(blk + 1024 + lane * 16);
            }
        }
        lds_wave_sync();
        const size_t base = (size_t)sub * 32 * ld * ELEM;
        for (int r = r0; r < 32; r += rstep) {
            if (sub * 32 + r >= M) break;
            const size_t off = base + (size_t)r * ld * ELEM + q * 16;
            typedef uint32_t u32x4 __attribute__((ext_vector_type(4)));
            if constexpr (ELEM == 4) {
                const f32x4 a = *reinterpret_cast<const f32x4*>(tile + r * pitch + q * 16);
                f32x4 d = *reinterpret_cast<const f32x4*>(delta + off);
                *reinterpret_cast<f32x4*>(act_out + off) = a;
#pragma unroll
                for (int e = 0; e < 4; ++e) { if (!(a[e] > 0.0f)) d[e] = 0.0f; acc[e] += d[e]; }
                *reinterpret_cast<f32x4*>(delta + off) = d;
            } else {
                const u32x4 a = *reinterpret_cast<const u32x4*>(tile + r * pitch + q * 16);
// ... 798 lines not shown
```

### nerf_amd/ops.py

```python
import ctypes as C
from typing import Optional, Sequence

import torch

from . import _lib
from ._lib import lib, check, Samples, F32, BF16, BF16_F8, NET_PROPOSAL, NET_MIP, NET_REF, NET_PROPOSAL_128, NET_MIP_128, PROP_W128, FINE_W128, ACT_RELU, ACT_IDENTITY, ACT_SOFTPLUS

_PRECISION_OVERRIDE = None


def set_precision(p: Optional[str]):
    global _PRECISION_OVERRIDE
    if p not in (None, "fp32", "bf16"):
        raise ValueError("precision must be None, 'fp32' or 'bf16'")
    _PRECISION_OVERRIDE = p


_TRAIN_DUMPS = __import__("os").environ.get("NERF_AMD_TRAIN_DUMPS", "bf16")


def set_train_dumps(fmt: str):
    global _TRAIN_DUMPS
    if fmt not in ("bf16", "fp8"):
        raise ValueError("train dumps: 'bf16' or 'fp8'")
# ... 662 lines not shown
                    seed: Optional[int] = None, rng_ray_offset: int = 0, contract: bool = False):
    in_kernel_rng = u_strat is None
    if in_kernel_rng:
        if u_inv is not None or seed is None:
            raise ValueError("nerf_amd: u_strat and u_inv are both tensors, or both None with a `seed`")
        dev = rays.device if rays is not None else z_base.device
        if camera is None:
            camera = Samples()
        camera.rng_seed, camera.rng_ray_offset = int(seed) & 0xFFFFFFFFFFFFFFFF, int(rng_ray_offset)
    else:
        dev = u_strat.device
    if contract:
        if camera is None:
            camera = Samples()
        camera.contract = 1
    N = n_rays if n_rays is not None else (rays.shape[0] if in_kernel_rng else u_strat.shape[0])
    need = lib.nerf_amd_render_ref_workspace_bytes(N, n_fine)
    if workspace is None or workspace.numel() < need:
        workspace = torch.empty(need, dtype=torch.uint8, device=dev)
    rgb = torch.empty((N, 3), dtype=torch.float32, device=dev)
    depth = torch.empty((N,), dtype=torch.float32, device=dev) if want_depth else None
    cam_dir = _dev(cam_dir, "cam_dir") if cam_dir is not None else None
    normal_img = torch.empty((N,), dtype=torch.float32, device=dev) if cam_dir is not None else None
    check(lib.nerf_amd_render_rays_ref(_ptr(packed_prop), _ptr(packed_ref), _prop_prec(packed_prop, precision), int(flags), _ptr(rays),
                                       C.byref(camera) if camera is not None else None, ray_offset, _ptr(z_base), _ptr(u_strat),
                                       _ptr(u_inv), N, n_fine, float(near), float(far), int(white_bkg), _ptr(cam_dir), _ptr(rgb),
                                       _ptr(depth), _ptr(normal_img), _ptr(workspace), _stream()), "nerf_amd_render_rays_ref")
    return rgb, depth, normal_img, workspace


BWD_MAX_SAMPLES = 1024


def sigma_to_weights_backward(sigma: torch.Tensor, z: torch.Tensor, dirs: Optional[torch.Tensor], act: int, d_weights: torch.Tensor) -> torch.Tensor:
    sigma, z, d_weights = _dev(sigma, "density"), _dev(z, "zvals"), _dev(d_weights, "d_weights")
    dirs = _dev(dirs, "ray_dirs") if dirs is not None else None
    N, S = sigma.shape
    out = torch.empty_like(sigma)
    check(lib.nerf_amd_sigma_to_weights_backward(_ptr(sigma), _ptr(z), _ptr(dirs), N, S, act, _ptr(d_weights), _ptr(out), _stream()),
          "nerf_amd_sigma_to_weights_backward")
    return out


def composite_backward(rgbo: torch.Tensor, z: torch.Tensor, dirs: torch.Tensor, mul_norm: bool, white_bkg: bool, act: int, near_far,
                       d_rgb: Optional[torch.Tensor], d_weights: Optional[torch.Tensor], d_depth: Optional[torch.Tensor],
                       sigma_shift: float = 0.0) -> torch.Tensor:
    rgbo, z = _dev(rgbo, "rgbo"), _dev(z, "depth")
    N, S = rgbo.shape[0], rgbo.shape[1]
    if dirs.shape[-1] == 6:
        dirs = _dev(dirs, "rays")
        dirs_ptr, dirs_stride = C.c_void_p(dirs.data_ptr() + 12), 6
    else:
        dirs = _dev(dirs, "ray_dirs")
        dirs_ptr, dirs_stride = _ptr(dirs), 3
    d_rgb = _dev(d_rgb, "d_rgb") if d_rgb is not None else torch.zeros((N, 3), dtype=torch.float32, device=rgbo.device)
    d_weights = _dev(d_weights, "d_weights") if d_weights is not None else None
    d_depth = _dev(d_depth, "d_depth") if d_depth is not None else None
    near, far = (near_far if near_far is not None else (0.0, 1.0))
    out = torch.empty_like(rgbo)
    flags = (1 if mul_norm else 0) | (2 if white_bkg else 0)
    check(lib.nerf_amd_composite_backward(_ptr(rgbo), _ptr(z), z.shape[-1], dirs_ptr, dirs_stride, N, S, flags, act, float(sigma_shift),
                                          float(near), float(far), _ptr(d_rgb), _ptr(d_weights), _ptr(d_depth), _ptr(out), _stream()),
          "nerf_amd_composite_backward")
    return out


def max_blur_backward(weights: torch.Tensor, d_out: torch.Tensor) -> torch.Tensor:
    weights, d_out = _dev(weights, "weights"), _dev(d_out, "d_out")
    S = weights.shape[-1]
    out = torch.empty_like(weights)
    check(lib.nerf_amd_max_blur_backward(_ptr(weights), _ptr(d_out), weights.numel() // S, S, _ptr(out), _stream()), "nerf_amd_max_blur_backward")
    return out


def get_bounds_backward(below: torch.Tensor, d_bounds: torch.Tensor, n_coarse: int) -> torch.Tensor:
    d_bounds = _dev(d_bounds, "d_bounds")
    below = below.to(torch.int64).contiguous()
    N, K = below.shape
    out = torch.empty((N, n_coarse), dtype=torch.float32, device=d_bounds.device)
    check(lib.nerf_amd_get_bounds_backward(_ptr(below), _ptr(d_bounds), N, n_coarse, K, _ptr(out), _stream()), "nerf_amd_get_bounds_backward")
    return out


NET_PROPOSAL, NET_MIP = 0, 1


def _train_forward_samples(net: int, packed: torch.Tensor, precision: int, s: Samples, out_shape, device):
    out = torch.empty(out_shape, dtype=torch.float32, device=device)
    dump = leased(("dump", net), lib.nerf_amd_train_dump_bytes(net, precision, s.M), device)
    if s.M:
        fn = lib.nerf_amd_proposal_forward_train if net == NET_PROPOSAL else lib.nerf_amd_mip_forward_train
        check(fn(_ptr(packed), precision, C.byref(s), _ptr(out), _ptr(dump), _stream()), "nerf_amd_*_forward_train")
    return out, dump


def proposal_forward_train(packed: torch.Tensor, precision: int, pts: torch.Tensor, contract: bool = False):
    pts = _dev(pts, "pts")
    return _train_forward_samples(NET_PROPOSAL, packed, precision, _samples_pts(pts, 3, contract), pts.shape[:-1], pts.device)


def mip_forward_train(packed: torch.Tensor, precision: int, pts: torch.Tensor, contract: bool = False):
    pts = _dev(pts, "pts")
    return _train_forward_samples(NET_MIP, packed, precision, _samples_pts(pts, 6, contract), pts.shape[:-1] + (4,), pts.device)


def mip_forward_train_samples(packed: torch.Tensor, precision: int, s: Samples, shape, device):
    return _train_forward_samples(NET_MIP, packed, precision, s, tuple(shape) + (4,), device)


def proposal_forward_train_samples(packed: torch.Tensor, precision: int, s: Samples, shape, device):
    return _train_forward_samples(NET_PROPOSAL, packed, precision, s, tuple(shape), device)


def train_dump_rows(dump: torch.Tensor, net: int, precision: int, M: int, layer: int, n_features: int) -> torch.Tensor:
    out = torch.empty((M, n_features), dtype=torch.bfloat16 if precision == BF16 else torch.float32, device=dump.device)
    check(lib.nerf_amd_train_dump_to_rows(_ptr(dump), net, precision, M, layer, n_features, _ptr(out), _stream()), "nerf_amd_train_dump_to_rows")
    return out


def train_dump_rows_mask_(dump: torch.Tensor, net: int, precision: int, layer: int, delta: torch.Tensor):
    assert delta.is_contiguous() and delta.dim() == 2 and delta.dtype == (torch.bfloat16 if precision == BF16 else torch.float32)
    M, F = delta.shape
    act = torch.empty_like(delta)
    part = torch.empty((lib.nerf_amd_train_dump_rows_mask_partials(), F), dtype=torch.float32, device=delta.device)
    check(lib.nerf_amd_train_dump_rows_mask(_ptr(dump), net, precision, M, layer, F, _ptr(act), _ptr(delta), _ptr(part), _stream()),
          "nerf_amd_train_dump_rows_mask")
    return act, delta, part.sum(0)


def encode_rows(x: torch.Tensor, L: int, precision: int, normalize: bool = False) -> torch.Tensor:
    if not x.is_cuda:
        raise RuntimeError("nerf_amd: 'x' must live on the HIP device (got %s); there is no CPU path" % x.device)
    if x.dtype != torch.float32 or x.dim() != 2 or x.stride(1) != 1 or x.shape[1] < 3:
        x = x.reshape(-1, x.shape[-1]).float().contiguous()
    M = x.shape[0]
    out = torch.empty((M, (3 + 6 * L + 7) // 8 * 8), dtype=torch.bfloat16 if precision == BF16 else torch.float32, device=x.device)
    check(lib.nerf_amd_encode_rows(_ptr(x), max(x.stride(0), 3), M, L, int(normalize), precision, _ptr(out), _stream()), "nerf_amd_encode_rows")
    return out


def relu_mask_(delta: torch.Tensor, act: torch.Tensor, precision: int) -> torch.Tensor:
    assert delta.is_contiguous() and act.is_contiguous() and delta.shape == act.shape and delta.dtype == act.dtype
    check(lib.nerf_amd_relu_mask(_ptr(delta), _ptr(act), precision, delta.numel(), _stream()), "nerf_amd_relu_mask")
    return delta


def relu_mask_bias_(delta: torch.Tensor, act: torch.Tensor, precision: int):
    assert delta.is_contiguous() and act.is_contiguous() and delta.shape == act.shape and delta.dtype == act.dtype and delta.dim() == 2
    n_part = lib.nerf_amd_relu_mask_bias_partials(precision, delta.shape[0], delta.shape[1])
    part = torch.empty((n_part, delta.shape[1]), dtype=torch.float32, device=delta.device)
    check(lib.nerf_amd_relu_mask_bias(_ptr(delta), _ptr(act), precision, delta.shape[0], delta.shape[1], _ptr(part), _stream()), "nerf_amd_relu_mask_bias")
    return delta, part.sum(0)



def _ptr_array(tensors):
    return (C.c_void_p * len(tensors))(*[t.data_ptr() for t in tensors])


def pack_weights_backward(net: int, precision: int, weights: Sequence[torch.Tensor]) -> torch.Tensor:
    ws = [_raw(w, "weight") for w in weights]
    blob = torch.empty(lib.nerf_amd_packed_backward_bytes(net, precision), dtype=torch.uint8, device=ws[0].device)
    check(lib.nerf_amd_pack_weights_backward(net, precision, _ptr_array(ws), len(ws), _ptr(blob), _stream()), "nerf_amd_pack_weights_backward")
    return blob


# ... 333 lines not shown
```

### nerf_amd/training.py

```python
from typing import Optional, Tuple

import torch
import torch.nn.functional as F

from . import ops
from .addtional import DistortionLoss, ProposalLoss, ProposalNetwork, getBounds
from .mip_methods import maxBlurFilter
from .nerf_base import NeRF
from .optim import Adam
from .utils import _focal_xy, crop_window, inverseSample, randomFromOneImage

_M62 = (1 << 62) - 1


def rank_seed(seed: int, rank: int) -> int:
    seed, rank = int(seed), int(rank)
    if not 0 <= rank <= _M62:
        raise ValueError("nerf_amd.training.rank_seed: rank must be in [0, 2^62)")
    if rank == 0:
        return seed
    x = rank
    x = ((x ^ (x >> 31)) * 0xBF58476D1CE4E5B9) & _M62
    x = ((x ^ (x >> 29)) * 0x94D049BB133111EB) & _M62
    x ^= x >> 32
    return (seed & _M62) ^ x


class TrainStep:
    def __init__(self, prop_net, mip_net, optimizer: Adam, image_hw: Tuple[int, int], focal, near: float, far: float, ray_num: int = 512,
                 coarse_pnum: int = 64, fine_pnum: int = 128, crop_xy=(1.0, 1.0), seed: Optional[int] = None, white_bkg: bool = False,
                 prop_normal: bool = False, grad_hook=None, ipe_radius: Optional[float] = None, contract: bool = False, flat_grads=None,
                 *, scene=None, view_ids=None, grad_clip: float = -0.01, distortion: float = 0.0):
        if not isinstance(optimizer, Adam) or not optimizer.lr_on_device:
            raise ValueError("nerf_amd.training.TrainStep needs nerf_amd.optim.Adam(..., lr_on_device=True): the step must not read host state")
        self.prop_net, self.mip_net, self.opt = prop_net, mip_net, optimizer
        self.near, self.far, self.ray_num, self.coarse_pnum, self.fine_pnum = float(near), float(far), int(ray_num), int(coarse_pnum), int(fine_pnum)
        self.fx, self.fy = _focal_xy(focal)
        self.white_bkg = bool(white_bkg)
        from .ref_model import RefNeRF
        self.is_ref = isinstance(mip_net, RefNeRF)
        self.ipe_radius, self.contract = (None if ipe_radius is None else float(ipe_radius)), bool(contract)
        if self.is_ref and self.ipe_radius is not None:
            raise NotImplementedError("nerf_amd.training.TrainStep: the integrated PE is wired for the MipNeRF branch (the Ref-NeRF kernel encodes points)")
        self.distortion = float(distortion)
        if not self.distortion >= 0.0:
            raise ValueError("nerf_amd.training.TrainStep: distortion must be >= 0")
        if self.is_ref and self.distortion > 0.0:
            raise NotImplementedError("nerf_amd.training.TrainStep: the distortion loss is wired for the MipNeRF branch (the Ref-NeRF step's merged "
                                      "sample set has no closed last interval)")
        self.prop_normal = bool(prop_normal) and self.is_ref
        dev = next(mip_net.parameters()).device
        H, W = image_hw
        self.image_hw = (int(H), int(W))
        self.scene = None
        if scene is None:
            if view_ids is not None:
                raise ValueError("nerf_amd.training.TrainStep: view_ids needs scene=(images, poses)")
            self.image = torch.zeros((3, H, W), dtype=torch.float32, device=dev)
            self.pose = torch.zeros((3, 4), dtype=torch.float32, device=dev)
        else:
            images, poses = scene
            for t, name in ((images, "images"), (poses, "poses")):
                if not (isinstance(t, torch.Tensor) and t.is_cuda and t.dtype == torch.float32 and t.is_contiguous() and t.device == dev):
                    raise ValueError("nerf_amd.training.TrainStep: scene %s must be a contiguous fp32 tensor on the networks' device" % name)
            if images.dim() != 4 or images.shape[1] != 3 or poses.dim() != 3 or tuple(poses.shape) != (images.shape[0], 3, 4):
                raise ValueError("nerf_amd.training.TrainStep: scene = (images (V,3,H,W), poses (V,3,4)), got %s and %s"
                                 % (tuple(images.shape), tuple(poses.shape)))
            if tuple(images.shape[2:]) != self.image_hw:
                raise ValueError("nerf_amd.training.TrainStep: image_hw %s is not the scene's %s" % (self.image_hw, tuple(images.shape[2:])))
            self.scene = (images, poses)
            self.view_ids = ops.scene_view_ids(view_ids, images.shape[0], dev)
            self.ray_index = torch.zeros((self.ray_num,), dtype=torch.int64, device=dev)
            self.image = self.pose = None
        self.crop_xy = tuple(crop_xy)
        if seed is None:
            seed = int(torch.randint(0, 2 ** 62, (1,)).item())
        if self.scene is not None and flat_grads is not None and flat_grads is not False:
            import torch.distributed as dist
            if dist.is_available() and dist.is_initialized() and dist.get_world_size(flat_grads.group) > 1:
                seed = rank_seed(seed, dist.get_rank(flat_grads.group))
        self.seed = torch.full((1,), seed, dtype=torch.int64, device=dev)
        self.loss = torch.zeros((), dtype=torch.float32, device=dev)
        self.img_loss = torch.zeros((), dtype=torch.float32, device=dev)
        self.dist_loss = torch.zeros((), dtype=torch.float32, device=dev)
        self.dist_fn = DistortionLoss(self.distortion / (self.far - self.near)) if self.distortion > 0.0 else None
        if self.is_ref:
            mip_net.__dict__["noise_seed_dev"] = self.seed
        self.prop_loss_fn = ProposalLoss()
        self.grad_hook = grad_hook
        self._reduce = flat_grads is not None and flat_grads is not False
        if flat_grads is None:
            from .parallel import FlatGradients
            owner = mip_net.__dict__.get("_grad_owner")
            if owner is not None and prop_net.__dict__.get("_grad_owner") is owner and owner.covers([mip_net, prop_net]):
                flat_grads = owner
            else:
                flat_grads = FlatGradients([mip_net, prop_net], optimizer)
        self.flat_grads = flat_grads if flat_grads is not False else None
        if self.flat_grads is not None and getattr(self.flat_grads, "_dead", False):
            raise ValueError("nerf_amd.training.TrainStep: the FlatGradients passed in was detached by a newer owner of these modules")
        self.grad_clip = float(grad_clip)
        self.graph = None

    def release(self) -> None:
        net = getattr(self, "mip_net", None)
        if net is not None and getattr(self, "is_ref", False) and net.__dict__.get("noise_seed_dev") is getattr(self, "seed", None):
            net.__dict__.pop("noise_seed_dev", None)

    def __del__(self):
        try:
            self.release()
        except Exception:
            pass

    def _body(self):
        if self.scene is not None:
            pts, z_c, rgb_tgt, rays, _ = ops.sample_scene_rays(self.scene[0], self.scene[1], self.fx, self.fy, self.near, self.far, self.ray_num,
                                                               self.coarse_pnum, seed_dev=self.seed, window=crop_window(*self.image_hw, self.crop_xy),
                                                               view_ids=self.view_ids, index_out=self.ray_index)
        else:
            pixels, coords = randomFromOneImage(self.image, self.crop_xy)
            pts, z_c, rgb_tgt, rays = ops.sample_training_rays_dev(pixels, coords, self.pose, self.fx, self.fy, self.near, self.far, self.ray_num,
                                                                   self.coarse_pnum, self.seed)
        dirs = rays[:, 3:]
        if self.prop_normal:
            pts.requires_grad_(True)
        density = self.prop_net.forward(pts, contract=True) if self.contract else self.prop_net.forward(pts)
        if self.prop_normal:
            from .ref_model import RefNeRF
            coarse_grad = -RefNeRF.get_grad(density, pts)
        density = F.softplus(density)
        prop_w = maxBlurFilter(ProposalNetwork.get_weights(density, z_c, dirs), 0.01)
        u = ops.philox_uniforms((self.ray_num, self.fine_pnum + 1), seed_dev=self.seed)
        z_f, below = inverseSample(prop_w, z_c, self.fine_pnum + 1, sort=True, u=u)
        extra = 0.0
        if self.is_ref:
            from .ref_model import BackFaceLoss, RefNeRF, WeightedNormalLoss
            samples, z_f, below, sort_ids = NeRF.coarseFineMerge(rays, z_c, z_f, below)
            pos, fine_dir = samples.split((3, 3), dim=-1)
            pos.requires_grad_(True)
            rgbo, pred_normal = self.mip_net.forward(pos, fine_dir, contract=True) if self.contract else self.mip_net.forward(pos, fine_dir)
            density_grad = -RefNeRF.get_grad(rgbo[..., -1], pos)
            rgbo[..., -1] = F.softplus(rgbo[..., -1] + 0.5)
            rendered, weights, _ = NeRF.render(rgbo, z_f, dirs, self.mip_net.density_act, white_bkg=self.white_bkg)
            extra = 4e-4 * WeightedNormalLoss()(weights, density_grad, pred_normal) + 0.1 * BackFaceLoss()(weights, pred_normal, fine_dir)
            if self.prop_normal:
                picked = RefNeRF.coarse_grad_select(density_grad, sort_ids, self.coarse_pnum)
                extra = extra + 4e-5 * WeightedNormalLoss()(prop_w, picked.detach(), coarse_grad)
        else:
            edges = z_f
            if self.ipe_radius is not None:
                rgbo = self.mip_net.forward_rays(rays, z_f, self.fine_pnum, ipe_radius=self.ipe_radius, contract=self.contract)
                z_f = z_f[..., :-1].contiguous()
            else:
                z_f = z_f[..., :-1].contiguous()
                rgbo = (self.mip_net.forward_rays(rays, z_f, self.fine_pnum, contract=True) if self.contract
                        else self.mip_net.forward(NeRF.length2pts(rays, z_f)))
            rendered, weights, _ = NeRF.render(rgbo, z_f, dirs, white_bkg=self.white_bkg)
            if self.dist_fn is not None:
                extra = self.dist_fn(weights, edges)
        bounds = getBounds(prop_w, below)
        if self.flat_grads is not None:
            self.flat_grads.bind(); self.flat_grads.begin_step()
        else:
            self.opt.zero_grad(set_to_none=True)
        img_loss = torch.mean((rendered - rgb_tgt) ** 2)
        loss = self.prop_loss_fn(bounds, weights.detach()) + img_loss + extra
        loss.backward()
        if self._reduce:
            self.flat_grads.all_reduce()
        if self.grad_hook is not None:
            self.grad_hook()
        if self.grad_clip > 0.0:
            if self.flat_grads is not None:
                self.flat_grads.finalize_window()
                flat = self.flat_grads.flat
                flat.mul_(torch.clamp(self.grad_clip / (torch.linalg.vector_norm(flat) + 1e-6), max=1.0))
            else:
                torch.nn.utils.clip_grad_norm_(list(self.mip_net.parameters()) + list(self.prop_net.parameters()), self.grad_clip)
        self.opt.step()
        ops.advance_seed(self.seed)
        self.loss.copy_(loss.detach())
        self.img_loss.copy_(img_loss.detach())
        if self.dist_fn is not None:
            self.dist_loss.copy_(extra.detach())

    def set_image(self, img: torch.Tensor, pose: torch.Tensor) -> None:
        if self.scene is not None:
            raise ValueError("nerf_amd.training.TrainStep: a scene-mode step draws from the whole stack and takes no image")
        self.image.copy_(img.reshape(self.image.shape), non_blocking=True)
        self.pose.copy_(pose.reshape(-1)[:12].reshape(3, 4), non_blocking=True)

    def set_crop(self, crop_xy) -> None:
        crop_xy = tuple(crop_xy)
        if crop_xy != self.crop_xy:
            self.crop_xy = crop_xy
            self.graph = None

    def capture(self, warmup: int = 2) -> None:
        if self.grad_hook is not None:
            raise RuntimeError("nerf_amd.training.TrainStep: an iteration with a grad_hook (collective) is not captured; run it eagerly")
        self.prop_net.train(); self.mip_net.train()
        for _ in range(max(1, warmup)):
            self._body()
        torch.cuda.synchronize()
        self.graph = torch.cuda.CUDAGraph()
        kw = {}
        if self._reduce and torch.distributed.is_available() and torch.distributed.is_initialized():
            if torch.distributed.get_backend(self.flat_grads.group) != "nccl":
                raise RuntimeError("nerf_amd.training.TrainStep: only an RCCL (backend 'nccl') all-reduce can be captured into the hipGraph")
            kw["capture_error_mode"] = "thread_local"
        with torch.cuda.graph(self.graph, **kw):
            self._body()

    def __call__(self, img: Optional[torch.Tensor] = None, pose: Optional[torch.Tensor] = None):
        if img is not None:
            self.set_image(img, pose)
        if self.graph is not None:
            self.opt.sync_lr()
            self.graph.replay()
            ops.parameters_changed()
        else:
            self._body()
        return self.loss, self.img_loss
```

Measured before the change: 9.507 million.

## Fuse training tail into coarse-to-fine and render-losses HIP kernels

Adds three HIP kernels. One turns proposal densities into weights and inverse-CDF fine samples and points. One is its backward. One composites the fine samples and produces the image and proposal losses together with their gradients in a single pass. TrainStep gains a default-on fused_tail path that uses these kernels in place of the chain of small PyTorch and autograd ops for the proposal and render losses. The aim is to cut kernel launches and intermediate tensor traffic in the training step. The cost is duplicated logic, size limits on coarse and fine sample counts, and a separate path that only applies to the non-ref, non-contract configuration without distortion loss.

```diff
diff --git a/include/nerf_amd.h b/include/nerf_amd.h
--- a/include/nerf_amd.h
+++ b/include/nerf_amd.h
@@ -206,6 +206,18 @@
 int nerf_amd_max_blur_backward(const float* weights, const float* d_out, int64_t N, int S, float* d_weights, void* stream);
 int nerf_amd_get_bounds_backward(const int64_t* below, const float* d_bounds, int64_t N, int C, int K, float* d_w_prop, void* stream);
 
+#define NERF_AMD_COARSE_TO_FINE_MAX 256
+int nerf_amd_coarse_to_fine(const float* density, const float* z, const float* rays, const float* dir_norm, uint64_t seed, const uint64_t* seed_dev,
+                            int64_t N, int C, int K, float alpha, float* prop_w, float* z_fine, int64_t* below, float* z_fine_c, float* pts,
+                            void* stream);
+int nerf_amd_proposal_weights_backward(const float* density, const float* z, const float* rays, const float* dir_norm, const float* g, int64_t N,
+                                       int C, float* d_density, void* stream);
+#define NERF_AMD_RENDER_LOSSES_MAX_F 128
+#define NERF_AMD_RENDER_LOSSES_WORKSPACE_FLOATS 16384
+int nerf_amd_render_losses(const float* rgbo, const float* z, int z_stride, const float* dirs, int dirs_stride, const float* rgb_tgt,
+                           const float* prop_w, const int64_t* below, int64_t N, int C, int F, int white_bkg, float* rendered, float* weights,
+                           float* bounds, float* d_rgbo, float* d_prop_w, float* losses, float* workspace, void* stream);
+
 size_t nerf_amd_render_workspace_bytes(int64_t N, int n_fine);
 int    nerf_amd_render_rays(const void* packed_prop, const void* packed_mip, int precision,
                             const float* rays, const nerf_amd_samples* camera, int64_t ray_offset,
diff --git a/nerf_amd/_lib.py b/nerf_amd/_lib.py
--- a/nerf_amd/_lib.py
+++ b/nerf_amd/_lib.py
@@ -111,6 +111,11 @@
                                               C.c_float, c_void, c_void, c_void, c_void, c_void]),
     "nerf_amd_max_blur_backward": (C.c_int, [c_void, c_void, i64, C.c_int, c_void, c_void]),
     "nerf_amd_get_bounds_backward": (C.c_int, [c_void, c_void, i64, C.c_int, C.c_int, c_void, c_void]),
+    "nerf_amd_coarse_to_fine": (C.c_int, [c_void, c_void, c_void, c_void, C.c_uint64, c_void, i64, C.c_int, C.c_int, C.c_float, c_void, c_void, c_void, c_void,
+                                          c_void, c_void]),
+    "nerf_amd_proposal_weights_backward": (C.c_int, [c_void, c_void, c_void, c_void, c_void, i64, C.c_int, c_void, c_void]),
+    "nerf_amd_render_losses": (C.c_int, [c_void, c_void, C.c_int, c_void, C.c_int, c_void, c_void, c_void, i64, C.c_int, C.c_int, C.c_int, c_void, c_void,
+                                         c_void, c_void, c_void, c_void, c_void, c_void]),
     "nerf_amd_render_workspace_bytes": (C.c_size_t, [i64, C.c_int]),
     "nerf_amd_render_rays": (C.c_int, [c_void, c_void, C.c_int, c_void, C.POINTER(Samples), i64, c_void, c_void, c_void, i64,
                                        C.c_int, C.c_float, C.c_float, C.c_int, c_void, c_void, c_void, c_void, c_void]),
diff --git a/nerf_amd/csrc/capi.hip b/nerf_amd/csrc/capi.hip
--- a/nerf_amd/csrc/capi.hip
+++ b/nerf_amd/csrc/capi.hip
@@ -93,6 +93,11 @@
                         const float*, const float*, int, float, float, float*, int, int, float*, hipStream_t);
 int sk_max_blur_backward(const float*, const float*, int64_t, int, float*, hipStream_t);
 int sk_get_bounds_backward(const int64_t*, const float*, int64_t, int, int, float*, hipStream_t);
+int tt_coarse_to_fine(const float*, const float*, const float*, const float*, uint64_t, const uint64_t*, int64_t, int, int, float, float*, float*, int64_t*,
+                      float*, float*, hipStream_t);
+int tt_proposal_weights_backward(const float*, const float*, const float*, const float*, const float*, int64_t, int, float*, hipStream_t);
+int tt_render_losses(const float*, const float*, int, const float*, int, const float*, const float*, const int64_t*, int64_t, int, int, int, float*, float*,
+                     float*, float*, float*, float*, float*, hipStream_t);
 
 namespace {
 thread_local char g_err[512] = "";
@@ -405,6 +410,34 @@
     if (N < 0 || C < 1 || C > 4096 || K < 2) return fail(NERF_AMD_EINVAL, "bad size");
     if (N && (!w_prop || !below || !bounds)) return fail(NERF_AMD_EINVAL, "NULL argument");
     return hip_status(sk_get_bounds(w_prop, below, N, C, K, bounds, S(stream)), "nerf_amd_get_bounds");
+}
+
+int nerf_amd_coarse_to_fine(const float* density, const float* z, const float* rays, const float* dir_norm, uint64_t seed, const uint64_t* seed_dev,
+                            int64_t N, int C, int K, float alpha, float* prop_w, float* z_fine, int64_t* below, float* z_fine_c, float* pts,
+                            void* stream) {
+    if (N < 0 || C < 3 || C > NERF_AMD_COARSE_TO_FINE_MAX || K < 2 || K > NERF_AMD_COARSE_TO_FINE_MAX + 1)
+        return fail(NERF_AMD_EINVAL, "bad size (3 <= C <= 256 coarse samples, 2 <= K <= 257 fine depths: four rays' rows live in 64 KiB of LDS)");
+    if (N && (!density || !z || !rays || !prop_w || !z_fine || !below)) return fail(NERF_AMD_EINVAL, "NULL argument");
+    return hip_status(tt_coarse_to_fine(density, z, rays, dir_norm, seed, seed_dev, N, C, K, alpha, prop_w, z_fine, below, z_fine_c, pts, S(stream)),
+                      "nerf_amd_coarse_to_fine");
+}
+
+int nerf_amd_proposal_weights_backward(const float* density, const float* z, const float* rays, const float* dir_norm, const float* g, int64_t N,
+                                       int C, float* d_density, void* stream) {
+    if (N < 0 || C < 1 || C > NERF_AMD_COARSE_TO_FINE_MAX) return fail(NERF_AMD_EINVAL, "bad size (1 <= C <= 256 coarse samples: a ray lives in registers)");
+    if (N && (!density || !z || !rays || !g || !d_density)) return fail(NERF_AMD_EINVAL, "NULL argument");
+    return hip_status(tt_proposal_weights_backward(density, z, rays, dir_norm, g, N, C, d_density, S(stream)), "nerf_amd_proposal_weights_backward");
+}
+
+int nerf_amd_render_losses(const float* rgbo, const float* z, int z_stride, const float* dirs, int dirs_stride, const float* rgb_tgt,
+                           const float* prop_w, const int64_t* below, int64_t N, int C, int F, int white_bkg, float* rendered, float* weights,
+                           float* bounds, float* d_rgbo, float* d_prop_w, float* losses, float* workspace, void* stream) {
+    if (N < 1 || C < 1 || C > 4096 || F < 1 || F > NERF_AMD_RENDER_LOSSES_MAX_F || z_stride < F || dirs_stride < 3)
+        return fail(NERF_AMD_EINVAL, "bad size or stride (N >= 1, 1 <= C <= 4096, 1 <= F <= 128 fine samples per ray: a ray lives in registers)");
+    if (!rgbo || !z || !dirs || !rgb_tgt || !prop_w || !below || !rendered || !d_rgbo || !d_prop_w || !losses || !workspace)
+        return fail(NERF_AMD_EINVAL, "NULL argument");
+    return hip_status(tt_render_losses(rgbo, z, z_stride, dirs, dirs_stride, rgb_tgt, prop_w, below, N, C, F, white_bkg, rendered, weights, bounds,
+                                       d_rgbo, d_prop_w, losses, workspace, S(stream)), "nerf_amd_render_losses");
 }
 
 int nerf_amd_merge_depths(const float* z_fine, const float* z_coarse, int64_t N, int K, int C, float* z_out, void* stream) {
diff --git a/nerf_amd/csrc/ray_stages.h b/nerf_amd/csrc/ray_stages.h
--- /dev/null
+++ b/nerf_amd/csrc/ray_stages.h
@@ -0,0 +1,306 @@
+#pragma once
+#include "device_common.h"
+
+constexpr int WAVES_PER_BLOCK = 4;
+
+DEVINL int wave_in_block() { return (int)(threadIdx.x >> 6); }
+
+DEVINL void lds_wave_sync() {
+    __builtin_amdgcn_fence(__ATOMIC_RELEASE, "workgroup");
+    __builtin_amdgcn_wave_barrier();
+    __builtin_amdgcn_fence(__ATOMIC_ACQUIRE, "workgroup");
+}
+
+DEVINL void wave_bounds_sat(const float* __restrict__ w_row, int C, float* sat) {
+    const int lane = lane_id();
+    double carry = 0.0;
+    if (lane == 0) sat[0] = 0.0f;
+    for (int base = 0; base < C; base += 64) {
+        const int j = base + lane;
+        const double p = (j < C) ? (double)w_row[j] : 0.0;
+        const double incl = wave_incl_scan_add(p);
+        if (j < C) sat[1 + j] = (float)(carry + incl);
+        carry += wave_last(incl);
+    }
+}
+DEVINL float bounds_from_sat(const float* sat, int st, int en) { return sat[en] - sat[st]; }
+
+DEVINL void wave_bounds_backward(const int* bl, const float* g, int C, int K, float* __restrict__ dw_row) {
+    for (int j = lane_id(); j < C; j += 64) {
+        float acc = 0.0f;
+        for (int k = 0; k < K - 1; ++k) {
+            const int st = bl[k];
+            int en = bl[k + 1] + 1;
+            en = en > C ? C : en;
+            if (j >= st && j < en) acc += g[k];
+            else if (j >= en && j < st) acc -= g[k];
+        }
+        dw_row[j] = acc;
+    }
+}
+DEVINL int clamp_below(int64_t b, int C) { return b < 0 ? 0 : (b > C ? C : (int)b); }
+
+struct WeightsBwdArgs {
+    const float* sigma; int sigma_stride;
+    int sigma_off;
+    const float* z; int z_stride; const float* dirs; int dirs_stride; int64_t N; int S; int mul_norm; int act; float sigma_shift;
+    const float* rgbo; const float* d_rgb; const float* d_weights; const float* d_depth; int white_bkg; float near, far;
+    float* d_sigma; int d_sigma_stride; int d_sigma_off; float* d_rgbo;
+};
+DEVINL float density_act_grad(float x, int act) {
+    if (act == 0) return x > 0.0f ? 1.0f : 0.0f;
+    if (act == 2) return x > 20.0f ? 1.0f : 1.0f / (1.0f + expf(-x));
+    return 1.0f;
+}
+template <int BWD_CHUNKS>
+DEVINL void wave_weights_backward(const WeightsBwdArgs& a, int64_t n, float dr, float dg, float db, float dd_) {
+    const int S = a.S;
+    const int lane = lane_id();
+    float nrm = 1.0f;
+    if (a.mul_norm && a.dirs) { const float* dd = a.dirs + n * a.dirs_stride; nrm = norm3(dd[0], dd[1], dd[2]); }
+    const float* zz = a.z + n * a.z_stride;
+    const float bg = a.white_bkg ? ((dr + dg) + db) : 0.0f;
+    float m[BWD_CHUNKS], T[BWD_CHUNKS], G[BWD_CHUNKS], delta[BWD_CHUNKS], x[BWD_CHUNKS];
+    double carry = 1.0, gw_carry = 0.0;
+    double P[BWD_CHUNKS];
+#pragma unroll
+    for (int c = 0; c < BWD_CHUNKS; ++c) {
+        const int s = c * 64 + lane;
+        const bool ok = s < S;
+        m[c] = 1.0f; T[c] = 0.0f; G[c] = 0.0f; delta[c] = 0.0f; x[c] = 0.0f;
+        double p = 1.0;
+        float zn0 = 0.0f;
+        if (c * 64 < S) {
+            if (ok) {
+                zn0 = zz[s] * nrm;
+                delta[c] = (s + 1 < S) ? (zz[s + 1] * nrm - zn0) : 1e10f;
+                x[c] = a.sigma[(n * S + s) * a.sigma_stride + a.sigma_off] + a.sigma_shift;
+                m[c] = expf(-density_act(x[c], a.act) * delta[c]);
+                p = (double)(m[c] + 1e-10f);
+            }
+            const double incl = wave_incl_scan_mul(p);
+            const double excl = wave_shift_up1(incl, 1.0);
+            T[c] = (float)(carry * excl);
+            carry *= wave_last(incl);
+            float g = 0.0f;
+            if (ok) {
+                if (a.d_weights) g += a.d_weights[n * S + s];
+                if (a.rgbo) {
+                    const float* cc = a.rgbo + (n * S + s) * 4;
+                    g += ((dr * cc[0] + dg * cc[1]) + db * cc[2]) - bg;
+                }
+                g += dd_ * zn0;
+            }
+            G[c] = g;
+            const float w = (1.0f - m[c]) * T[c];
+            const double gi = wave_incl_scan_add(ok ? (double)(g * w) : 0.0);
+            P[c] = gw_carry + gi;
+            gw_carry += wave_last(gi);
+            if (ok && a.d_rgbo) {
+                float* o = a.d_rgbo + (n * S + s) * 4;
+                o[0] = w * dr; o[1] = w * dg; o[2] = w * db;
+            }
+        }
+    }
+    const double total = gw_carry;
+#pragma unroll
+    for (int c = 0; c < BWD_CHUNKS; ++c) {
+        const int s = c * 64 + lane;
+        if (s < S) {
+            const float suffix = (float)(total - P[c]);
+            const float dm = -G[c] * T[c] + suffix / (m[c] + 1e-10f);
+            const float ds = dm * (-delta[c] * m[c]) * density_act_grad(x[c], a.act);
+            a.d_sigma[(n * S + s) * a.d_sigma_stride + a.d_sigma_off] = ds;
+        }
+    }
+}
+
+DEVINL float max_blur_at(const float* w, int s, int S, float alpha) {
+    const float c = w[s];
+    const float front = (s == 0) ? c : fmaxf(w[s - 1], c);
+    const float rear = (s == S - 1) ? c : fmaxf(c, w[s + 1]);
+    return 0.5f * (front + rear) + alpha;
+}
+DEVINL float max_blur_backward_at(const float* w, const float* g, int s, int S) {
+    const float c = w[s];
+    float acc = 0.0f;
+    if (s == 0) acc += 0.5f * g[s];
+    if (s == S - 1) acc += 0.5f * g[s];
+    if (s + 1 < S) {
+        const float o = w[s + 1];
+        const float share = c > o ? 1.0f : (c == o ? 0.5f : 0.0f);
+        acc += share * (0.5f * g[s] + 0.5f * g[s + 1]);
+    }
+    if (s >= 1) {
+        const float o = w[s - 1];
+        const float share = c > o ? 1.0f : (c == o ? 0.5f : 0.0f);
+        acc += share * (0.5f * g[s - 1] + 0.5f * g[s]);
+    }
+    return acc;
+}
+DEVINL float length2pts_at(const float* r, int k, float z) { return (k < 3) ? (r[k] + r[3 + k] * z) : r[k]; }
+
+#ifndef SORT_NB_DEF
+#define SORT_NB_DEF 256
+#define SORT_CAP_DEF 6
+#endif
+constexpr int SORT_NB = SORT_NB_DEF, SORT_CAP = SORT_CAP_DEF, SORT_PER_LANE = SORT_NB / 64;
+constexpr int SORT_LDS_FLOATS = 2 * SORT_NB + SORT_NB * SORT_CAP / 2;
+
+template <class UF>
+DEVINL void wave_inverse_sample(const float* pw, const float* bins, int nw, float* cdf, float* samp, int* bel, int* sortbuf,
+                                UF&& uf, int K, int sort, float* __restrict__ z_out,
+                                int64_t* __restrict__ below_out, int64_t* __restrict__ above_out) {
+    const int lane = lane_id();
+    const int nb = nw + 1;
+    float* part8 = reinterpret_cast<float*>(sortbuf);
+    const int nv = nw >> 3;
+    if (lane < 8) {
+        const int n4 = nv >> 2;
+        float a0 = 0.0f, a1 = 0.0f, a2 = 0.0f, a3 = 0.0f;
+        for (int i = 0; i < n4; ++i) {
+            a0 += pw[32 * i + lane] + 1e-5f;
+            a1 += pw[32 * i + 8 + lane] + 1e-5f;
+            a2 += pw[32 * i + 16 + lane] + 1e-5f;
+            a3 += pw[32 * i + 24 + lane] + 1e-5f;
+        }
+        for (int v = 4 * n4; v < nv; ++v) a0 += pw[8 * v + lane] + 1e-5f;
+        a0 += a1; a0 += a2; a0 += a3;
+        part8[lane] = a0;
+    }
+    lds_wave_sync();
+    float total = 0.0f;
+    if (nv > 0) {
+        for (int j = 8 * nv; j < nw; ++j) total += pw[j] + 1e-5f;
+#pragma unroll
+        for (int c = 0; c < 8; ++c) total += part8[c];
+    } else {
+        float a1 = 0.0f, a2 = 0.0f, a3 = 0.0f;
+        if (nw >= 4) { total += pw[0] + 1e-5f; a1 += pw[1] + 1e-5f; a2 += pw[2] + 1e-5f; a3 += pw[3] + 1e-5f; }
+        for (int j = nw & ~3; j < nw; ++j) total += pw[j] + 1e-5f;
+        total += a1; total += a2; total += a3;
+    }
+    double carry = 0.0;
+    if (lane == 0) cdf[0] = 0.0f;
+    for (int base = 0; base < nw; base += 64) {
+        const int j = base + lane;
+        double p = 0.0;
+        if (j < nw) p = (double)((pw[j] + 1e-5f) / total);
+        const double incl = wave_incl_scan_add(p);
+        if (j < nw) cdf[1 + j] = (float)(carry + incl);
+        carry += wave_last(incl);
+    }
+    lds_wave_sync();
+    const int halvings = 32 - __builtin_clz((unsigned)nb);
+    for (int k0 = 0, i0 = 0; k0 < K; k0 += 192, i0 += 3) {
+        float uu[3]; int lo[3], hi[3];
+#pragma unroll
+        for (int q = 0; q < 3; ++q) {
+            const int k = k0 + 64 * q + lane;
+            uu[q] = (k < K) ? uf(i0 + q, k) : 0.0f;
+            lo[q] = 0; hi[q] = (k < K) ? nb : 0;
+        }
+        for (int it = 0; it < halvings; ++it) {
+#pragma unroll
+            for (int q = 0; q < 3; ++q) {
+                const int mid = (lo[q] + hi[q]) >> 1;
+                const bool open_ = lo[q] < hi[q];
+                const float c = cdf[open_ ? mid : 0];
+                if (open_) { if (c <= uu[q]) lo[q] = mid + 1; else hi[q] = mid; }
+            }
+        }
+#pragma unroll
+        for (int q = 0; q < 3; ++q) {
+            const int k = k0 + 64 * q + lane;
+            if (k >= K) continue;
+            const int below = lo[q] - 1 > 0 ? lo[q] - 1 : 0;
+            const int above = lo[q] < nb - 1 ? lo[q] : nb - 1;
+            const float c0 = cdf[below], c1 = cdf[above];
+            float denom = c1 - c0;
+            if (denom < 1e-5f) denom = 1.0f;
+            const float t = (uu[q] - c0) / denom;
+            const float b0 = bins[below], b1 = bins[above];
+            const float v = b0 + t * (b1 - b0);
+            if (sort) { samp[k] = v; bel[k] = below; }
+            else {
+                z_out[k] = v;
+                if (below_out) below_out[k] = below;
+                if (above_out) above_out[k] = above;
+            }
+        }
+    }
+    if (!sort) return;
+    lds_wave_sync();
+    int* cnt = sortbuf;
+    int* pre = sortbuf + SORT_NB;
+    unsigned short* mem = reinterpret_cast<unsigned short*>(sortbuf + 2 * SORT_NB);
+    for (int b = lane; b < SORT_NB; b += 64) cnt[b] = 0;
+    lds_wave_sync();
+    int overflow = 0;
+    for (int j = lane; j + 1 < nb; j += 64) overflow |= (bins[j + 1] < bins[j]) ? 1 : 0;
+    for (int k = lane, i = 0; k < K; k += 64, ++i) {
+        int b = (int)(uf(i, k) * (float)SORT_NB);
+        b = b < 0 ? 0 : (b > SORT_NB - 1 ? SORT_NB - 1 : b);
+        const int pos = atomicAdd(&cnt[b], 1);
+        if (pos < SORT_CAP) mem[b * SORT_CAP + pos] = (unsigned short)k; else overflow = 1;
+    }
+    lds_wave_sync();
+    if (__any(overflow)) {
+        for (int k = lane; k < K; k += 64) {
+            const float v = samp[k];
+            int rank = 0;
+            for (int j = 0; j < K; ++j) {
+                const float o = samp[j];
+                rank += (o < v || (o == v && j < k)) ? 1 : 0;
+            }
+            z_out[rank] = v;
+            if (below_out) below_out[rank] = bel[k];
+        }
+        return;
+    }
+    {
+        int c[SORT_PER_LANE], tot = 0;
+#pragma unroll
+        for (int i = 0; i < SORT_PER_LANE; ++i) { c[i] = cnt[lane * SORT_PER_LANE + i]; tot += c[i]; }
+        int run = wave_incl_scan_add(tot) - tot;
+#pragma unroll
+        for (int i = 0; i < SORT_PER_LANE; ++i) { pre[lane * SORT_PER_LANE + i] = run; run += c[i]; }
+    }
+    lds_wave_sync();
+    for (int k0 = 0, i0 = 0; k0 < K; k0 += 192, i0 += 3) {
+        float v[3]; int rank[3], cntb[3], bb[3];
+#pragma unroll
+        for (int q = 0; q < 3; ++q) {
+            const int k = k0 + 64 * q + lane;
+            const bool ok = k < K;
+            int b = ok ? (int)(uf(i0 + q, k) * (float)SORT_NB) : 0;
+            b = b < 0 ? 0 : (b > SORT_NB - 1 ? SORT_NB - 1 : b);
+            bb[q] = b;
+            v[q] = samp[ok ? k : 0];
+            rank[q] = pre[b];
+            cntb[q] = ok ? cnt[b] : 0;
+        }
+        int most = cntb[0] > cntb[1] ? cntb[0] : cntb[1];
+        most = most > cntb[2] ? most : cntb[2];
+        const int trips = wave_max_i(most);
+        for (int p = 0; p < trips; ++p) {
+#pragma unroll
+            for (int q = 0; q < 3; ++q) {
+                const int k = k0 + 64 * q + lane;
+                const bool live = p < cntb[q];
+                const int jx = mem[bb[q] * SORT_CAP + p];
+                const float o = samp[live ? jx : 0];
+                rank[q] += (live && (o < v[q] || (o == v[q] && jx < k))) ? 1 : 0;
+            }
+        }
+#pragma unroll
+        for (int q = 0; q < 3; ++q) {
+            const int k = k0 + 64 * q + lane;
+            if (k >= K) continue;
+            z_out[rank[q]] = v[q];
+            if (below_out) below_out[rank[q]] = bel[k];
+        }
+    }
+}
+
+DEVINL size_t inv_lds_floats(int C, int K) { return (size_t)3 * C + 2 * K + SORT_LDS_FLOATS; }
diff --git a/nerf_amd/csrc/sample_kernels.hip b/nerf_amd/csrc/sample_kernels.hip
--- a/nerf_amd/csrc/sample_kernels.hip
+++ b/nerf_amd/csrc/sample_kernels.hip
@@ -1,14 +1,11 @@
 #include "device_common.h"
+#include "ray_stages.h"
 #include "host_common.h"
 #include "../../include/nerf_amd.h"
 
 extern __shared__ __attribute__((aligned(16))) char smem[];
 
 namespace {
-
-constexpr int WAVES_PER_BLOCK = 4;
-
-DEVINL int wave_in_block() { return (int)(threadIdx.x >> 6); }
 
 constexpr int ENC_TILE = 64;
 static inline size_t enc_lds_bytes(int L) { return (size_t)ENC_TILE * (6 * L + 6) * 4; }
@@ -281,7 +278,7 @@
         const int k = (int)(i - ns * 6);
         const int64_t n = ns / S;
         const float* r = rays + n * 6;
-        out[i] = (k < 3) ? (r[k] + r[3 + k] * z[ns]) : r[k];
+        out[i] = length2pts_at(r, k, z[ns]);
     }
 }
 
@@ -305,183 +302,9 @@
     const int64_t total = N * S;
     for (int64_t i = blockIdx.x * (int64_t)blockDim.x + threadIdx.x; i < total; i += (int64_t)gridDim.x * blockDim.x) {
         const int s = (int)(i % S);
-        const float c = w[i];
-        const float front = (s == 0) ? c : fmaxf(w[i - 1], c);
-        const float rear = (s == S - 1) ? c : fmaxf(c, w[i + 1]);
-        out[i] = 0.5f * (front + rear) + alpha;
-    }
-}
-
-DEVINL void lds_wave_sync() {
-    __builtin_amdgcn_fence(__ATOMIC_RELEASE, "workgroup");
-    __builtin_amdgcn_wave_barrier();
-    __builtin_amdgcn_fence(__ATOMIC_ACQUIRE, "workgroup");
-}
-
-#ifndef SORT_NB_DEF
-#define SORT_NB_DEF 256
-#define SORT_CAP_DEF 6
-#endif
-constexpr int SORT_NB = SORT_NB_DEF, SORT_CAP = SORT_CAP_DEF, SORT_PER_LANE = SORT_NB / 64;
-constexpr int SORT_LDS_FLOATS = 2 * SORT_NB + SORT_NB * SORT_CAP / 2;
-
-template <class UF>
-DEVINL void wave_inverse_sample(const float* pw, const float* bins, int nw, float* cdf, float* samp, int* bel, int* sortbuf,
-                                UF&& uf, int K, int sort, float* __restrict__ z_out,
-                                int64_t* __restrict__ below_out, int64_t* __restrict__ above_out) {
-    const int lane = lane_id();
-    const int nb = nw + 1;
-    float* part8 = reinterpret_cast<float*>(sortbuf);
-    const int nv = nw >> 3;
-    if (lane < 8) {
-        const int n4 = nv >> 2;
-        float a0 = 0.0f, a1 = 0.0f, a2 = 0.0f, a3 = 0.0f;
-        for (int i = 0; i < n4; ++i) {
-            a0 += pw[32 * i + lane] + 1e-5f;
-            a1 += pw[32 * i + 8 + lane] + 1e-5f;
-            a2 += pw[32 * i + 16 + lane] + 1e-5f;
-            a3 += pw[32 * i + 24 + lane] + 1e-5f;
-        }
-        for (int v = 4 * n4; v < nv; ++v) a0 += pw[8 * v + lane] + 1e-5f;
-        a0 += a1; a0 += a2; a0 += a3;
-        part8[lane] = a0;
-    }
-    lds_wave_sync();
-    float total = 0.0f;
-    if (nv > 0) {
-        for (int j = 8 * nv; j < nw; ++j) total += pw[j] + 1e-5f;
-#pragma unroll
-        for (int c = 0; c < 8; ++c) total += part8[c];
-    } else {
-        float a1 = 0.0f, a2 = 0.0f, a3 = 0.0f;
-        if (nw >= 4) { total += pw[0] + 1e-5f; a1 += pw[1] + 1e-5f; a2 += pw[2] + 1e-5f; a3 += pw[3] + 1e-5f; }
-        for (int j = nw & ~3; j < nw; ++j) total += pw[j] + 1e-5f;
-        total += a1; total += a2; total += a3;
-    }
-    double carry = 0.0;
-    if (lane == 0) cdf[0] = 0.0f;
-    for (int base = 0; base < nw; base += 64) {
-        const int j = base + lane;
-        double p = 0.0;
-        if (j < nw) p = (double)((pw[j] + 1e-5f) / total);
-        const double incl = wave_incl_scan_add(p);
-        if (j < nw) cdf[1 + j] = (float)(carry + incl);
-        carry += wave_last(incl);
-    }
-    lds_wave_sync();
-    const int halvings = 32 - __builtin_clz((unsigned)nb);
-    for (int k0 = 0, i0 = 0; k0 < K; k0 += 192, i0 += 3) {
-        float uu[3]; int lo[3], hi[3];
-#pragma unroll
-        for (int q = 0; q < 3; ++q) {
-            const int k = k0 + 64 * q + lane;
-            uu[q] = (k < K) ? uf(i0 + q, k) : 0.0f;
-            lo[q] = 0; hi[q] = (k < K) ? nb : 0;
-        }
-        for (int it = 0; it < halvings; ++it) {
-#pragma unroll
-            for (int q = 0; q < 3; ++q) {
-                const int mid = (lo[q] + hi[q]) >> 1;
-                const bool open_ = lo[q] < hi[q];
-                const float c = cdf[open_ ? mid : 0];
-                if (open_) { if (c <= uu[q]) lo[q] = mid + 1; else hi[q] = mid; }
-            }
-        }
-#pragma unroll
-        for (int q = 0; q < 3; ++q) {
-            const int k = k0 + 64 * q + lane;
-            if (k >= K) continue;
-            const int below = lo[q] - 1 > 0 ? lo[q] - 1 : 0;
-            const int above = lo[q] < nb - 1 ? lo[q] : nb - 1;
-            const float c0 = cdf[below], c1 = cdf[above];
-            float denom = c1 - c0;
-            if (denom < 1e-5f) denom = 1.0f;
-            const float t = (uu[q] - c0) / denom;
-            const float b0 = bins[below], b1 = bins[above];
-            const float v = b0 + t * (b1 - b0);
-            if (sort) { samp[k] = v; bel[k] = below; }
-            else {
-                z_out[k] = v;
-                if (below_out) below_out[k] = below;
-                if (above_out) above_out[k] = above;
-            }
-        }
-    }
-    if (!sort) return;
-    lds_wave_sync();
-    int* cnt = sortbuf;
-    int* pre = sortbuf + SORT_NB;
-    unsigned short* mem = reinterpret_cast<unsigned short*>(sortbuf + 2 * SORT_NB);
-    for (int b = lane; b < SORT_NB; b += 64) cnt[b] = 0;
-    lds_wave_sync();
-    int overflow = 0;
-    for (int j = lane; j + 1 < nb; j += 64) overflow |= (bins[j + 1] < bins[j]) ? 1 : 0;
-    for (int k = lane, i = 0; k < K; k += 64, ++i) {
-        int b = (int)(uf(i, k) * (float)SORT_NB);
-        b = b < 0 ? 0 : (b > SORT_NB - 1 ? SORT_NB - 1 : b);
-        const int pos = atomicAdd(&cnt[b], 1);
-        if (pos < SORT_CAP) mem[b * SORT_CAP + pos] = (unsigned short)k; else overflow = 1;
-    }
-    lds_wave_sync();
-    if (__any(overflow)) {
-        for (int k = lane; k < K; k += 64) {
-            const float v = samp[k];
-            int rank = 0;
-            for (int j = 0; j < K; ++j) {
-                const float o = samp[j];
-                rank += (o < v || (o == v && j < k)) ? 1 : 0;
-            }
-            z_out[rank] = v;
-            if (below_out) below_out[rank] = bel[k];
-        }
-        return;
-    }
-    {
-        int c[SORT_PER_LANE], tot = 0;
-#pragma unroll
-        for (int i = 0; i < SORT_PER_LANE; ++i) { c[i] = cnt[lane * SORT_PER_LANE + i]; tot += c[i]; }
-        int run = wave_incl_scan_add(tot) - tot;
-#pragma unroll
-        for (int i = 0; i < SORT_PER_LANE; ++i) { pre[lane * SORT_PER_LANE + i] = run; run += c[i]; }
-    }
-    lds_wave_sync();
-    for (int k0 = 0, i0 = 0; k0 < K; k0 += 192, i0 += 3) {
-        float v[3]; int rank[3], cntb[3], bb[3];
-#pragma unroll
-        for (int q = 0; q < 3; ++q) {
-            const int k = k0 + 64 * q + lane;
-            const bool ok = k < K;
-            int b = ok ? (int)(uf(i0 + q, k) * (float)SORT_NB) : 0;
-            b = b < 0 ? 0 : (b > SORT_NB - 1 ? SORT_NB - 1 : b);
-            bb[q] = b;
-            v[q] = samp[ok ? k : 0];
-            rank[q] = pre[b];
-            cntb[q] = ok ? cnt[b] : 0;
-        }
-        int most = cntb[0] > cntb[1] ? cntb[0] : cntb[1];
-        most = most > cntb[2] ? most : cntb[2];
-        const int trips = wave_max_i(most);
-        for (int p = 0; p < trips; ++p) {
-#pragma unroll
-            for (int q = 0; q < 3; ++q) {
-                const int k = k0 + 64 * q + lane;
-                const bool live = p < cntb[q];
-                const int jx = mem[bb[q] * SORT_CAP + p];
-                const float o = samp[live ? jx : 0];
-                rank[q] += (live && (o < v[q] || (o == v[q] && jx < k))) ? 1 : 0;
-            }
-        }
-#pragma unroll
-        for (int q = 0; q < 3; ++q) {
-            const int k = k0 + 64 * q + lane;
-            if (k >= K) continue;
-            z_out[rank[q]] = v[q];
-            if (below_out) below_out[rank[q]] = bel[k];
-        }
-    }
-}
-
-DEVINL size_t inv_lds_floats(int C, int K) { return (size_t)3 * C + 2 * K + SORT_LDS_FLOATS; }
+        out[i] = max_blur_at(w + (i - s), s, S, alpha);
+    }
+}
 
 __global__ __launch_bounds__(256) void inverse_sample_kernel(const float* __restrict__ w, const float* __restrict__ z,
                                                             const float* __restrict__ u, int64_t N, int C, int K, int sort,
@@ -737,102 +560,24 @@
     const int lane = lane_id();
     for (int64_t n = blockIdx.x * (int64_t)WAVES_PER_BLOCK + wave_in_block(); n < N; n += (int64_t)gridDim.x * WAVES_PER_BLOCK) {
         lds_wave_sync();
-        double carry = 0.0;
-        if (lane == 0) sat[0] = 0.0f;
-        for (int base = 0; base < C; base += 64) {
-            const int j = base + lane;
-            const double p = (j < C) ? (double)w[n * C + j] : 0.0;
-            const double incl = wave_incl_scan_add(p);
-            if (j < C) sat[1 + j] = (float)(carry + incl);
-            carry += wave_last(incl);
-        }
+        wave_bounds_sat(w + n * C, C, sat);
         lds_wave_sync();
         const int64_t* bl = below + n * K;
         for (int k = lane; k < K - 1; k += 64) {
             const int st = (int)bl[k], en = (int)bl[k + 1] + 1;
-            bounds[n * (K - 1) + k] = sat[en] - sat[st];
+            bounds[n * (K - 1) + k] = bounds_from_sat(sat, st, en);
         }
     }
 }
 
 constexpr int BWD_MAX_CHUNKS = 16;
-struct WeightsBwdArgs {
-    const float* sigma; int sigma_stride;
-    int sigma_off;
-    const float* z; int z_stride; const float* dirs; int dirs_stride; int64_t N; int S; int mul_norm; int act; float sigma_shift;
-    const float* rgbo; const float* d_rgb; const float* d_weights; const float* d_depth; int white_bkg; float near, far;
-    float* d_sigma; int d_sigma_stride; int d_sigma_off; float* d_rgbo;
-};
-DEVINL float density_act_grad(float x, int act) {
-    if (act == 0) return x > 0.0f ? 1.0f : 0.0f;
-    if (act == 2) return x > 20.0f ? 1.0f : 1.0f / (1.0f + expf(-x));
-    return 1.0f;
-}
 template <int BWD_CHUNKS>
 __global__ __launch_bounds__(256) void weights_backward_kernel(WeightsBwdArgs a) {
-    const int S = a.S;
-    const int lane = lane_id();
     for (int64_t n = blockIdx.x * (int64_t)WAVES_PER_BLOCK + wave_in_block(); n < a.N; n += (int64_t)gridDim.x * WAVES_PER_BLOCK) {
-        float nrm = 1.0f;
-        if (a.mul_norm && a.dirs) { const float* dd = a.dirs + n * a.dirs_stride; nrm = norm3(dd[0], dd[1], dd[2]); }
-        const float* zz = a.z + n * a.z_stride;
         float dr = 0.0f, dg = 0.0f, db = 0.0f, dd_ = 0.0f;
         if (a.d_rgb) { dr = a.d_rgb[n * 3]; dg = a.d_rgb[n * 3 + 1]; db = a.d_rgb[n * 3 + 2]; }
         if (a.d_depth) dd_ = a.d_depth[n] / (a.far - a.near);
-        const float bg = (a.white_bkg && a.d_rgb) ? ((dr + dg) + db) : 0.0f;
-        float m[BWD_CHUNKS], T[BWD_CHUNKS], G[BWD_CHUNKS], delta[BWD_CHUNKS], x[BWD_CHUNKS];
-        double carry = 1.0, gw_carry = 0.0;
-        double P[BWD_CHUNKS];
-#pragma unroll
-        for (int c = 0; c < BWD_CHUNKS; ++c) {
-            const int s = c * 64 + lane;
-            const bool ok = s < S;
-            m[c] = 1.0f; T[c] = 0.0f; G[c] = 0.0f; delta[c] = 0.0f; x[c] = 0.0f;
-            double p = 1.0;
-            float zn0 = 0.0f;
-            if (c * 64 < S) {
-                if (ok) {
-                    zn0 = zz[s] * nrm;
-                    delta[c] = (s + 1 < S) ? (zz[s + 1] * nrm - zn0) : 1e10f;
-                    x[c] = a.sigma[(n * S + s) * a.sigma_stride + a.sigma_off] + a.sigma_shift;
-                    m[c] = expf(-density_act(x[c], a.act) * delta[c]);
-                    p = (double)(m[c] + 1e-10f);
-                }
-                const double incl = wave_incl_scan_mul(p);
-                const double excl = wave_shift_up1(incl, 1.0);
-                T[c] = (float)(carry * excl);
-                carry *= wave_last(incl);
-                float g = 0.0f;
-                if (ok) {
-                    if (a.d_weights) g += a.d_weights[n * S + s];
-                    if (a.rgbo) {
-                        const float* cc = a.rgbo + (n * S + s) * 4;
-                        g += ((dr * cc[0] + dg * cc[1]) + db * cc[2]) - bg;
-                    }
-                    g += dd_ * zn0;
-                }
-                G[c] = g;
-                const float w = (1.0f - m[c]) * T[c];
-                const double gi = wave_incl_scan_add(ok ? (double)(g * w) : 0.0);
-                P[c] = gw_carry + gi;
-                gw_carry += wave_last(gi);
-                if (ok && a.d_rgbo) {
-                    float* o = a.d_rgbo + (n * S + s) * 4;
-                    o[0] = w * dr; o[1] = w * dg; o[2] = w * db;
-                }
-            }
-        }
-        const double total = gw_carry;
-#pragma unroll
-        for (int c = 0; c < BWD_CHUNKS; ++c) {
-            const int s = c * 64 + lane;
-            if (s < S) {
-                const float suffix = (float)(total - P[c]);
-                const float dm = -G[c] * T[c] + suffix / (m[c] + 1e-10f);
-                const float ds = dm * (-delta[c] * m[c]) * density_act_grad(x[c], a.act);
-                a.d_sigma[(n * S + s) * a.d_sigma_stride + a.d_sigma_off] = ds;
-            }
-        }
+        wave_weights_backward<BWD_CHUNKS>(a, n, dr, dg, db, dd_);
     }
 }
 
@@ -840,21 +585,7 @@
     const int64_t total = N * S;
     for (int64_t i = blockIdx.x * (int64_t)blockDim.x + threadIdx.x; i < total; i += (int64_t)gridDim.x * blockDim.x) {
         const int s = (int)(i % S);
-        const float c = w[i];
-        float acc = 0.0f;
-        if (s == 0) acc += 0.5f * g[i];
-        if (s == S - 1) acc += 0.5f * g[i];
-        if (s + 1 < S) {
-            const float o = w[i + 1];
-            const float share = c > o ? 1.0f : (c == o ? 0.5f : 0.0f);
-            acc += share * (0.5f * g[i] + 0.5f * g[i + 1]);
-        }
-        if (s >= 1) {
-            const float o = w[i - 1];
-            const float share = c > o ? 1.0f : (c == o ? 0.5f : 0.0f);
-            acc += share * (0.5f * g[i - 1] + 0.5f * g[i]);
-        }
-        dw[i] = acc;
+        dw[i] = max_blur_backward_at(w + (i - s), g + (i - s), s, S);
     }
 }
 
@@ -871,17 +602,7 @@
             g_lds[k] = (k < K - 1) ? g[n * (K - 1) + k] : 0.0f;
         }
         lds_wave_sync();
-        for (int j = lane; j < C; j += 64) {
-            float acc = 0.0f;
-            for (int k = 0; k < K - 1; ++k) {
-                const int st = bl_lds[k];
-                int en = bl_lds[k + 1] + 1;
-                en = en > C ? C : en;
-                if (j >= st && j < en) acc += g_lds[k];
-                else if (j >= en && j < st) acc -= g_lds[k];
-            }
-            dw[n * C + j] = acc;
-        }
+        wave_bounds_backward(bl_lds, g_lds, C, K, dw + n * C);
     }
 }
 
diff --git a/nerf_amd/csrc/train_tail_kernels.hip b/nerf_amd/csrc/train_tail_kernels.hip
--- /dev/null
+++ b/nerf_amd/csrc/train_tail_kernels.hip
@@ -0,0 +1,249 @@
+#include "device_common.h"
+#include "ray_stages.h"
+#include "host_common.h"
+#include "../../include/nerf_amd.h"
+
+extern __shared__ __attribute__((aligned(16))) char smem[];
+
+namespace {
+
+struct RenderLossArgs {
+    const float* rgbo; const float* z; int z_stride; const float* dirs; int dirs_stride; const float* rgb_tgt; const float* prop_w;
+    const int64_t* below; int64_t N; int C; int F; int white_bkg;
+    float* rendered; float* weights; float* bounds; float* d_rgbo; float* d_prop_w; double* partial;
+};
+constexpr int RL_BLOCKS = 4096;
+DEVINL size_t rl_lds_floats(int C, int F) { return (size_t)(C + 1) + F + 2 * (F + 1); }
+
+constexpr int RL_CHUNKS = 2;
+__global__ __launch_bounds__(256) void render_losses_kernel(RenderLossArgs a) {
+    const int C = a.C, F = a.F, K = a.F + 1, lane = lane_id();
+    float* sat = reinterpret_cast<float*>(smem) + wave_in_block() * rl_lds_floats(C, F);
+    float* wf = sat + (C + 1);
+    int* bl = reinterpret_cast<int*>(wf + F);
+    float* g = reinterpret_cast<float*>(bl + K);
+    const float inv_numel = 1.0f / (float)(3 * a.N);
+    double acc_prop = 0.0, acc_img = 0.0;
+    for (int64_t n = blockIdx.x * (int64_t)WAVES_PER_BLOCK + wave_in_block(); n < a.N; n += (int64_t)gridDim.x * WAVES_PER_BLOCK) {
+        lds_wave_sync();
+        wave_bounds_sat(a.prop_w + n * C, C, sat);
+        for (int k = lane; k < K; k += 64) bl[k] = clamp_below(a.below[n * K + k], C);
+        const float* dd = a.dirs + n * a.dirs_stride;
+        const float nrm = norm3(dd[0], dd[1], dd[2]);
+        const float* zz = a.z + n * a.z_stride;
+        const f32x4* px = reinterpret_cast<const f32x4*>(a.rgbo) + n * F;
+        float accr = 0.0f, accg = 0.0f, accb = 0.0f, accw = 0.0f;
+        float* wout = a.weights ? a.weights + n * F : nullptr;
+        wave_sigma_to_weights(F, NERF_AMD_ACT_RELU, [&](int s) { return px[s][3] + 0.0f; },
+                              [&](int s) { return zz[s] * nrm; },
+                              [&](int s, float w, float) {
+                                  const f32x4 c = px[s];
+                                  accr += w * c[0]; accg += w * c[1]; accb += w * c[2];
+                                  accw += w;
+                                  wf[s] = w;
+                                  if (wout) wout[s] = w;
+                              });
+        accr = wave_sum(accr); accg = wave_sum(accg); accb = wave_sum(accb); accw = wave_sum(accw);
+        if (a.white_bkg) { const float bg = 1.0f - accw; accr += bg; accg += bg; accb += bg; }
+        const float* tg = a.rgb_tgt + n * 3;
+        const float er = accr - tg[0], eg = accg - tg[1], eb = accb - tg[2];
+        const float dr = inv_numel * (2.0f * er), dg = inv_numel * (2.0f * eg), db = inv_numel * (2.0f * eb);
+        if (lane == 0) {
+            a.rendered[n * 3] = accr; a.rendered[n * 3 + 1] = accg; a.rendered[n * 3 + 2] = accb;
+            acc_img += ((double)er * (double)er + (double)eg * (double)eg) + (double)eb * (double)eb;
+        }
+        lds_wave_sync();
+        for (int k = lane; k < K; k += 64) {
+            float gb = 0.0f;
+            if (k < F) {
+                int en = bl[k + 1] + 1;
+                en = en > C ? C : en;
+                const float b = bounds_from_sat(sat, bl[k], en);
+                const float w = wf[k];
+                const float d = w - b;
+                const float r = d > 0.0f ? d : 0.0f;
+                const float den = w + 1e-8f;
+                const float gr = (1.0f / den) * (2.0f * r);
+                gb = -(r > 0.0f ? gr : 0.0f);
+                acc_prop += (double)r * (double)r / ((double)w + 1e-8);
+                if (a.bounds) a.bounds[n * F + k] = b;
+            }
+            g[k] = gb;
+        }
+        lds_wave_sync();
+        wave_bounds_backward(bl, g, C, K, a.d_prop_w + n * C);
+        WeightsBwdArgs wb{a.rgbo, 4, 3, a.z, a.z_stride, a.dirs, a.dirs_stride, a.N, F, 1, NERF_AMD_ACT_RELU, 0.0f, a.rgbo, nullptr, nullptr, nullptr,
+                          a.white_bkg, 0.0f, 1.0f, a.d_rgbo, 4, 3, a.d_rgbo};
+        wave_weights_backward<RL_CHUNKS>(wb, n, dr, dg, db, 0.0f);
+    }
+    acc_prop = wave_sum_d(acc_prop);
+    acc_img = wave_sum_d(acc_img);
+    __syncthreads();
+    double* red = reinterpret_cast<double*>(smem);
+    if (lane == 0) { red[2 * wave_in_block()] = acc_prop; red[2 * wave_in_block() + 1] = acc_img; }
+    __syncthreads();
+    if (threadIdx.x == 0) {
+        a.partial[2 * blockIdx.x] = ((red[0] + red[2]) + red[4]) + red[6];
+        a.partial[2 * blockIdx.x + 1] = ((red[1] + red[3]) + red[5]) + red[7];
+    }
+}
+__global__ __launch_bounds__(256) void render_losses_final_kernel(const double* __restrict__ partial, int n, int64_t N, float* __restrict__ out) {
+    double p = 0.0, q = 0.0;
+    for (int i = threadIdx.x; i < n; i += 256) { p += partial[2 * i]; q += partial[2 * i + 1]; }
+    p = wave_sum_d(p);
+    q = wave_sum_d(q);
+    double* red = reinterpret_cast<double*>(smem);
+    if (lane_id() == 0) { red[2 * wave_in_block()] = p; red[2 * wave_in_block() + 1] = q; }
+    __syncthreads();
+    if (threadIdx.x == 0) {
+        const double P = ((red[0] + red[2]) + red[4]) + red[6], Q = (((red[1] + red[3]) + red[5]) + red[7]) / (3.0 * (double)N);
+        out[0] = (float)(P + Q);
+        out[1] = (float)Q;
+    }
+}
+
+
+struct CoarseToFineArgs {
+    const float* density; const float* z; const float* rays; const float* dir_norm; const uint64_t* seed_dev; uint64_t seed;
+    int64_t N; int C; int K; float alpha;
+    float* prop_w; float* z_fine; int64_t* below; float* z_fine_c; float* pts;
+};
+static inline size_t ctf_lds_floats(int C, int K) {
+    const size_t f = (size_t)2 * K + 5 * (size_t)C + 3 * (size_t)K + SORT_LDS_FLOATS;
+    return (f + 1) & ~(size_t)1;
+}
+template <bool UREG>
+__global__ __launch_bounds__(256) void coarse_to_fine_kernel(CoarseToFineArgs a, size_t per_wave) {
+    const int C = a.C, K = a.K, F = a.K - 1, lane = lane_id();
+    float* base = reinterpret_cast<float*>(smem) + wave_in_block() * per_wave;
+    int64_t* bs = reinterpret_cast<int64_t*>(base);
+    float* pw = base + 2 * K; float* bins = pw + C; float* cdf = bins + C; float* samp = cdf + C;
+    int* bel = reinterpret_cast<int*>(samp + K);
+    int* sortbuf = bel + K;
+    float* zl = reinterpret_cast<float*>(sortbuf + SORT_LDS_FLOATS);
+    float* wraw = zl + C;
+    float* zs = wraw + C;
+    const uint64_t seed = a.seed_dev ? a.seed_dev[0] : a.seed;
+    for (int64_t n = blockIdx.x * (int64_t)WAVES_PER_BLOCK + wave_in_block(); n < a.N; n += (int64_t)gridDim.x * WAVES_PER_BLOCK) {
+        lds_wave_sync();
+        const float* ry = a.rays + n * 6;
+        const float nrm = a.dir_norm ? a.dir_norm[n] : norm3(ry[3], ry[4], ry[5]);
+        for (int j = lane; j < C; j += 64) zl[j] = a.z[n * C + j];
+        float u0 = 0.0f, u1 = 0.0f, u2 = 0.0f;
+        if (UREG) {
+            const Philox4 blk = philox_ray_block(seed, n, lane);
+            u0 = u01_from_bits(blk.w[1]); u1 = u01_from_bits(blk.w[2]); u2 = u01_from_bits(blk.w[3]);
+        }
+        lds_wave_sync();
+        const float* sg = a.density + n * C;
+        wave_sigma_to_weights(C, NERF_AMD_ACT_RELU, [=](int s) { return softplus_f(sg[s]); },
+                              [=](int s) { return zl[s] * nrm; },
+                              [=](int s, float wv, float) { wraw[s] = wv; });
+        lds_wave_sync();
+        for (int j = lane; j < C; j += 64) {
+            const float wb = max_blur_at(wraw, j, C, a.alpha);
+            if (j >= 1 && j <= C - 2) pw[j - 1] = wb;
+            a.prop_w[n * C + j] = wb;
+        }
+        for (int j = lane; j < C - 1; j += 64) bins[j] = 0.5f * (zl[j + 1] + zl[j]);
+        lds_wave_sync();
+        wave_inverse_sample(pw, bins, C - 2, cdf, samp, bel, sortbuf,
+                            [=](int i, int k) {
+                                if (UREG) return i == 0 ? u0 : (i == 1 ? u1 : u2);
+                                return philox_u_inv(seed, n, k);
+                            },
+                            K, 1, zs, bs, nullptr);
+        lds_wave_sync();
+        for (int k = lane; k < K; k += 64) {
+            const float zv = zs[k];
+            a.z_fine[n * K + k] = zv;
+            a.below[n * K + k] = bs[k];
+            if (a.z_fine_c && k < F) a.z_fine_c[n * F + k] = zv;
+        }
+        if (a.pts) {
+            float* o = a.pts + n * F * 6;
+            for (int i = lane; i < F * 6; i += 64) {
+                const int ns = i / 6, k = i - ns * 6;
+                o[i] = length2pts_at(ry, k, zs[ns]);
+            }
+        }
+    }
+}
+
+struct ProposalBwdArgs {
+    const float* density; const float* z; const float* rays; const float* dir_norm; const float* g; int64_t N; int C;
+    float* d_density;
+};
+template <int CHUNKS>
+__global__ __launch_bounds__(256) void proposal_weights_backward_kernel(ProposalBwdArgs a) {
+    const int C = a.C, lane = lane_id();
+    float* dens = reinterpret_cast<float*>(smem) + wave_in_block() * (size_t)(5 * C);
+    float* zn = dens + C; float* wraw = zn + C; float* dw = wraw + C; float* ds = dw + C;
+    for (int64_t n = blockIdx.x * (int64_t)WAVES_PER_BLOCK + wave_in_block(); n < a.N; n += (int64_t)gridDim.x * WAVES_PER_BLOCK) {
+        lds_wave_sync();
+        const float* ry = a.rays + n * 6;
+        const float nrm = a.dir_norm ? a.dir_norm[n] : norm3(ry[3], ry[4], ry[5]);
+        for (int j = lane; j < C; j += 64) {
+            dens[j] = softplus_f(a.density[n * C + j]);
+            zn[j] = a.z[n * C + j] * nrm;
+        }
+        lds_wave_sync();
+        wave_sigma_to_weights(C, NERF_AMD_ACT_RELU, [=](int s) { return dens[s]; }, [=](int s) { return zn[s]; },
+                              [=](int s, float wv, float) { wraw[s] = wv; });
+        lds_wave_sync();
+        const float* gn = a.g + n * C;
+        for (int j = lane; j < C; j += 64) dw[j] = max_blur_backward_at(wraw, gn, j, C);
+        lds_wave_sync();
+        WeightsBwdArgs wb{dens, 1, 0, zn, C, nullptr, 0, 1, C, 0, NERF_AMD_ACT_RELU, 0.0f, nullptr, nullptr, dw, nullptr, 0, 0.0f, 1.0f, ds, 1, 0, nullptr};
+        wave_weights_backward<CHUNKS>(wb, 0, 0.0f, 0.0f, 0.0f, 0.0f);
+        lds_wave_sync();
+        for (int j = lane; j < C; j += 64) {
+            const float x = a.density[n * C + j];
+            const float e = expf(x);
+            a.d_density[n * C + j] = x > 20.0f ? ds[j] : ds[j] * e / (e + 1.0f);
+        }
+    }
+}
+
+}
+
+int tt_render_losses(const float* rgbo, const float* z, int z_stride, const float* dirs, int dirs_stride, const float* rgb_tgt, const float* prop_w,
+                     const int64_t* below, int64_t N, int C, int F, int white_bkg, float* rendered, float* weights, float* bounds, float* d_rgbo,
+                     float* d_prop_w, float* losses, float* workspace, hipStream_t st) {
+    int64_t nb = (N + WAVES_PER_BLOCK - 1) / WAVES_PER_BLOCK;
+    const int blocks = (int)(nb > RL_BLOCKS ? RL_BLOCKS : (nb < 1 ? 1 : nb));
+    size_t lds = (size_t)WAVES_PER_BLOCK * ((size_t)(C + 1) + F + 2 * (F + 1)) * 4;
+    if (lds < 64) lds = 64;
+    double* partial = reinterpret_cast<double*>(workspace);
+    RenderLossArgs a{rgbo, z, z_stride, dirs, dirs_stride, rgb_tgt, prop_w, below, N, C, F, white_bkg, rendered, weights, bounds, d_rgbo, d_prop_w, partial};
+    if (F > 64 * RL_CHUNKS) return (int)hipErrorInvalidValue;
+    hipLaunchKernelGGL(render_losses_kernel, dim3(blocks), dim3(256), lds, st, a);
+    hipLaunchKernelGGL(render_losses_final_kernel, dim3(1), dim3(256), 64, st, partial, blocks, N, losses);
+    return (int)hipGetLastError();
+}
+
+int tt_coarse_to_fine(const float* density, const float* z, const float* rays, const float* dir_norm, uint64_t seed, const uint64_t* seed_dev, int64_t N, int C,
+                      int K, float alpha, float* prop_w, float* z_fine, int64_t* below, float* z_fine_c, float* pts, hipStream_t st) {
+    if (N == 0) return 0;
+    CoarseToFineArgs a{density, z, rays, dir_norm, seed_dev, seed, N, C, K, alpha, prop_w, z_fine, below, z_fine_c, pts};
+    const size_t per_wave = ctf_lds_floats(C, K);
+    int64_t blocks = (N + WAVES_PER_BLOCK - 1) / WAVES_PER_BLOCK;
+    const int64_t cap = (int64_t)nerf_host::cu_count() * 16;
+    if (blocks > cap) blocks = cap;
+    if (K <= 192) hipLaunchKernelGGL(coarse_to_fine_kernel<true>, dim3((unsigned)blocks), dim3(256), WAVES_PER_BLOCK * per_wave * 4, st, a, per_wave);
+    else hipLaunchKernelGGL(coarse_to_fine_kernel<false>, dim3((unsigned)blocks), dim3(256), WAVES_PER_BLOCK * per_wave * 4, st, a, per_wave);
+    return (int)hipGetLastError();
+}
+int tt_proposal_weights_backward(const float* density, const float* z, const float* rays, const float* dir_norm, const float* g, int64_t N, int C,
+                                 float* d_density, hipStream_t st) {
+    if (N == 0) return 0;
+    if (C > 256) return (int)hipErrorInvalidValue;
+    ProposalBwdArgs a{density, z, rays, dir_norm, g, N, C, d_density};
+    int64_t blocks = (N + WAVES_PER_BLOCK - 1) / WAVES_PER_BLOCK;
+    const int64_t cap = (int64_t)nerf_host::cu_count() * 16;
+    if (blocks > cap) blocks = cap;
+    const size_t lds = (size_t)WAVES_PER_BLOCK * 5 * C * 4;
+    if (C <= 128) hipLaunchKernelGGL(proposal_weights_backward_kernel<2>, dim3((unsigned)blocks), dim3(256), lds, st, a);
+    else hipLaunchKernelGGL(proposal_weights_backward_kernel<4>, dim3((unsigned)blocks), dim3(256), lds, st, a);
+    return (int)hipGetLastError();
+}
diff --git a/nerf_amd/ops.py b/nerf_amd/ops.py
--- a/nerf_amd/ops.py
+++ b/nerf_amd/ops.py
@@ -768,6 +768,83 @@
     return out
 
 
+COARSE_TO_FINE_MAX = 256
+
+
+def _dir_norm(dir_norm: Optional[torch.Tensor], N: int) -> Optional[torch.Tensor]:
+    if dir_norm is None:
+        return None
+    dir_norm = _dev(dir_norm, "dir_norm").reshape(-1)
+    if dir_norm.numel() != N:
+        raise ValueError("nerf_amd: dir_norm must hold one norm per ray")
+    return dir_norm
+
+
+def coarse_to_fine(density: torch.Tensor, z: torch.Tensor, rays: torch.Tensor, n_depths: int, seed: int = 0, seed_dev: Optional[torch.Tensor] = None,
+                   dir_norm: Optional[torch.Tensor] = None, alpha: float = 0.01, want_pts: bool = True, want_contiguous: bool = False):
+    density, z, rays = _dev(density, "density"), _dev(z, "zvals"), _dev(rays, "rays")
+    N, Cn = density.shape
+    K = int(n_depths)
+    if tuple(z.shape) != (N, Cn) or tuple(rays.shape) != (N, 6):
+        raise ValueError("nerf_amd: coarse_to_fine shapes: density (N,C), z (N,C), rays (N,6)")
+    dir_norm = _dir_norm(dir_norm, N)
+    if seed_dev is not None and (not seed_dev.is_cuda or seed_dev.dtype != torch.int64):
+        raise ValueError("nerf_amd: seed_dev must be a 1-element int64 device tensor")
+    dev = density.device
+    prop_w = torch.empty((N, Cn), dtype=torch.float32, device=dev)
+    z_f = torch.empty((N, K), dtype=torch.float32, device=dev)
+    below = torch.empty((N, K), dtype=torch.int64, device=dev)
+    pts = torch.empty((N, K - 1, 6), dtype=torch.float32, device=dev) if want_pts else None
+    z_fc = torch.empty((N, K - 1), dtype=torch.float32, device=dev) if want_contiguous else None
+    check(lib.nerf_amd_coarse_to_fine(_ptr(density), _ptr(z), _ptr(rays), _ptr(dir_norm), C.c_uint64(int(seed) & (2 ** 64 - 1)), _ptr(seed_dev), N, Cn, K,
+                                      float(alpha), _ptr(prop_w), _ptr(z_f), _ptr(below), _ptr(z_fc), _ptr(pts), _stream()), "nerf_amd_coarse_to_fine")
+    return prop_w, z_f, below, pts, z_fc
+
+
+def proposal_weights_backward(g: torch.Tensor, density: torch.Tensor, z: torch.Tensor, rays: torch.Tensor,
+                              dir_norm: Optional[torch.Tensor] = None) -> torch.Tensor:
+    g, density, z, rays = _dev(g, "d_prop_w"), _dev(density, "density"), _dev(z, "zvals"), _dev(rays, "rays")
+    N, Cn = density.shape
+    if tuple(z.shape) != (N, Cn) or tuple(rays.shape) != (N, 6) or tuple(g.shape) != (N, Cn):
+        raise ValueError("nerf_amd: proposal_weights_backward shapes: g (N,C), density (N,C), z (N,C), rays (N,6)")
+    dir_norm = _dir_norm(dir_norm, N)
+    out = torch.empty_like(density)
+    check(lib.nerf_amd_proposal_weights_backward(_ptr(density), _ptr(z), _ptr(rays), _ptr(dir_norm), _ptr(g), N, Cn, _ptr(out), _stream()),
+          "nerf_amd_proposal_weights_backward")
+    return out
+
+
+RENDER_LOSSES_MAX_F = 128
+RENDER_LOSSES_WORKSPACE_FLOATS = 16384
+
+
+def render_losses(rgbo: torch.Tensor, z: torch.Tensor, rays: torch.Tensor, rgb_tgt: torch.Tensor, prop_w: torch.Tensor, below: torch.Tensor,
+                  white_bkg: bool, losses: Optional[torch.Tensor] = None, want_weights: bool = False, want_bounds: bool = False):
+    rgbo, rays, rgb_tgt, prop_w = _dev(rgbo, "rgbo"), _dev(rays, "rays"), _dev(rgb_tgt, "rgb_tgt"), _dev(prop_w, "prop_w")
+    if not (z.is_cuda and z.dtype == torch.float32 and z.dim() == 2 and z.stride(1) == 1):
+        raise ValueError("nerf_amd: render_losses needs fp32 device depths (N, >= F) with unit column stride")
+    N, Fn = rgbo.shape[0], rgbo.shape[1]
+    Cn = prop_w.shape[-1]
+    if not below.is_cuda or below.dtype != torch.int64 or not below.is_contiguous():
+        raise ValueError("nerf_amd: render_losses needs a contiguous int64 device tensor 'below'")
+    if (rgbo.dim() != 3 or rgbo.shape[2] != 4 or tuple(rays.shape) != (N, 6) or tuple(rgb_tgt.shape) != (N, 3) or tuple(prop_w.shape) != (N, Cn)
+            or tuple(below.shape) != (N, Fn + 1) or z.shape[0] != N or z.shape[1] < Fn):
+        raise ValueError("nerf_amd: render_losses shapes: rgbo (N,F,4), z (N,>=F), rays (N,6), rgb_tgt (N,3), prop_w (N,C), below (N,F+1)")
+    dev = rgbo.device
+    rendered = torch.empty((N, 3), dtype=torch.float32, device=dev)
+    d_rgbo = torch.empty_like(rgbo)
+    d_prop_w = torch.empty_like(prop_w)
+    w = torch.empty((N, Fn), dtype=torch.float32, device=dev) if want_weights else None
+    bounds = torch.empty((N, Fn), dtype=torch.float32, device=dev) if want_bounds else None
+    if losses is None:
+        losses = torch.empty((2,), dtype=torch.float32, device=dev)
+    ws = torch.empty((RENDER_LOSSES_WORKSPACE_FLOATS,), dtype=torch.float32, device=dev)
+    check(lib.nerf_amd_render_losses(_ptr(rgbo), _ptr(z), z.stride(0), C.c_void_p(rays.data_ptr() + 12), 6, _ptr(rgb_tgt), _ptr(prop_w), _ptr(below),
+                                     N, Cn, Fn, 1 if white_bkg else 0, _ptr(rendered), _ptr(w), _ptr(bounds), _ptr(d_rgbo), _ptr(d_prop_w),
+                                     _ptr(losses), _ptr(ws), _stream()), "nerf_amd_render_losses")
+    return rendered, d_rgbo, d_prop_w, losses, w, bounds
+
+
 NET_PROPOSAL, NET_MIP = 0, 1
 
 
diff --git a/nerf_amd/training.py b/nerf_amd/training.py
--- a/nerf_amd/training.py
+++ b/nerf_amd/training.py
@@ -3,6 +3,7 @@
 import torch
 import torch.nn.functional as F
 
+from . import autograd_bridge as ab
 from . import ops
 from .addtional import DistortionLoss, ProposalLoss, ProposalNetwork, getBounds
 from .mip_methods import maxBlurFilter
@@ -30,7 +31,7 @@
     def __init__(self, prop_net, mip_net, optimizer: Adam, image_hw: Tuple[int, int], focal, near: float, far: float, ray_num: int = 512,
                  coarse_pnum: int = 64, fine_pnum: int = 128, crop_xy=(1.0, 1.0), seed: Optional[int] = None, white_bkg: bool = False,
                  prop_normal: bool = False, grad_hook=None, ipe_radius: Optional[float] = None, contract: bool = False, flat_grads=None,
-                 *, scene=None, view_ids=None, grad_clip: float = -0.01, distortion: float = 0.0):
+                 *, scene=None, view_ids=None, fused_tail: bool = True, grad_clip: float = -0.01, distortion: float = 0.0):
         if not isinstance(optimizer, Adam) or not optimizer.lr_on_device:
             raise ValueError("nerf_amd.training.TrainStep needs nerf_amd.optim.Adam(..., lr_on_device=True): the step must not read host state")
         self.prop_net, self.mip_net, self.opt = prop_net, mip_net, optimizer
@@ -80,8 +81,8 @@
             if dist.is_available() and dist.is_initialized() and dist.get_world_size(flat_grads.group) > 1:
                 seed = rank_seed(seed, dist.get_rank(flat_grads.group))
         self.seed = torch.full((1,), seed, dtype=torch.int64, device=dev)
-        self.loss = torch.zeros((), dtype=torch.float32, device=dev)
-        self.img_loss = torch.zeros((), dtype=torch.float32, device=dev)
+        self._losses = torch.zeros((2,), dtype=torch.float32, device=dev)
+        self.loss, self.img_loss = self._losses[0], self._losses[1]
         self.dist_loss = torch.zeros((), dtype=torch.float32, device=dev)
         self.dist_fn = DistortionLoss(self.distortion / (self.far - self.near)) if self.distortion > 0.0 else None
         if self.is_ref:
@@ -100,6 +101,8 @@
         if self.flat_grads is not None and getattr(self.flat_grads, "_dead", False):
             raise ValueError("nerf_amd.training.TrainStep: the FlatGradients passed in was detached by a newer owner of these modules")
         self.grad_clip = float(grad_clip)
+        self.fused_tail = (bool(fused_tail) and not self.is_ref and self.ipe_radius is None and not self.contract and self.dist_fn is None
+                           and 1 <= self.fine_pnum <= ops.RENDER_LOSSES_MAX_F and 3 <= self.coarse_pnum <= ops.COARSE_TO_FINE_MAX)
         self.graph = None
 
     def release(self) -> None:
@@ -122,6 +125,8 @@
             pixels, coords = randomFromOneImage(self.image, self.crop_xy)
             pts, z_c, rgb_tgt, rays = ops.sample_training_rays_dev(pixels, coords, self.pose, self.fx, self.fy, self.near, self.far, self.ray_num,
                                                                    self.coarse_pnum, self.seed)
+        if self.fused_tail:
+            return self._fused_body(pts, z_c, rgb_tgt, rays)
         dirs = rays[:, 3:]
         if self.prop_normal:
             pts.requires_grad_(True)
@@ -160,13 +165,36 @@
             if self.dist_fn is not None:
                 extra = self.dist_fn(weights, edges)
         bounds = getBounds(prop_w, below)
-        if self.flat_grads is not None:
-            self.flat_grads.bind(); self.flat_grads.begin_step()
-        else:
-            self.opt.zero_grad(set_to_none=True)
+        self._open_gradients()
         img_loss = torch.mean((rendered - rgb_tgt) ** 2)
         loss = self.prop_loss_fn(bounds, weights.detach()) + img_loss + extra
         loss.backward()
+        self._finish_step()
+        self.loss.copy_(loss.detach())
+        self.img_loss.copy_(img_loss.detach())
+        if self.dist_fn is not None:
+            self.dist_loss.copy_(extra.detach())
+
+    def _fused_body(self, pts, z_c, rgb_tgt, rays):
+        density = self.prop_net.forward(pts)
+        dir_norm = rays[:, 3:].norm(dim=-1, keepdim=True)
+        K = self.fine_pnum + 1
+        prop_w, z_f, below, samples = ab.HipOp.apply(
+            lambda d, z, r, nrm: ops.coarse_to_fine(d, z, r, K, seed_dev=self.seed, dir_norm=nrm)[:4],
+            lambda g, d, z, r, nrm: (ops.proposal_weights_backward(g, d, z, r, nrm), None, None, None), 1, density, z_c, rays, dir_norm)
+        rgbo = self.mip_net.forward(samples)
+        self._open_gradients()
+        _, g_rgbo, g_prop_w, _, _, _ = ops.render_losses(rgbo.detach(), z_f, rays, rgb_tgt, prop_w.detach(), below, self.white_bkg, losses=self._losses)
+        torch.autograd.backward([rgbo, prop_w], [g_rgbo, g_prop_w])
+        self._finish_step()
+
+    def _open_gradients(self):
+        if self.flat_grads is not None:
+            self.flat_grads.bind(); self.flat_grads.begin_step()
+        else:
+            self.opt.zero_grad(set_to_none=True)
+
+    def _finish_step(self):
         if self._reduce:
             self.flat_grads.all_reduce()
         if self.grad_hook is not None:
@@ -180,10 +208,6 @@
                 torch.nn.utils.clip_grad_norm_(list(self.mip_net.parameters()) + list(self.prop_net.parameters()), self.grad_clip)
         self.opt.step()
         ops.advance_seed(self.seed)
-        self.loss.copy_(loss.detach())
-        self.img_loss.copy_(img_loss.detach())
-        if self.dist_fn is not None:
-            self.dist_loss.copy_(extra.detach())
 
     def set_image(self, img: torch.Tensor, pose: torch.Tensor) -> None:
         if self.scene is not None:
```

New measurement: 9.508 million (median of 6 runs). About the same (+0.0%).
